# traveller59/spconv

Measured on NVIDIA H100. Metric: active-voxels/sec fwd+bwd SubMConv3d 3^3 C=64, higher is better.
Workload: dtype fp16

## Files before the change

spconv_b200/csrc/api_gemm.cu:

```cuda
#include "gemm.cuh"
#include "peer.cuh"
#include <stdlib.h>

using namespace spx;

namespace spx {
int write_tile_masks(const uint32_t *mask, int64_t rows, int kv, uint32_t *out, cudaStream_t stream);
}

static bool force_simt() { return runtime_cfg().force_simt != 0; }
static bool force_tc() { return runtime_cfg().force_tc != 0; }

static int check_desc(const spx_gemm_desc *d, const char *who) {
    SPX_REQUIRE(d != nullptr, "%s: descriptor is NULL", who);
    SPX_REQUIRE(d->kv >= 1 && d->kv <= 128, "%s: kernel volume %d not in [1,128]", who, d->kv);
    SPX_REQUIRE(d->c_in >= 1 && d->c_out >= 1, "%s: bad channel counts %d -> %d", who, d->c_in, d->c_out);
    SPX_REQUIRE(d->n_in >= 0 && d->n_out >= 0, "%s: negative row counts", who);
    SPX_REQUIRE(d->n_in < 2147483647ll && d->n_out < 2147483647ll, "%s: row counts must fit in int32", who);
    SPX_REQUIRE(d->pair != nullptr || (d->n_in == 0 || d->n_out == 0), "%s: pair table is NULL", who);
    SPX_REQUIRE((d->tile_table == nullptr) == (d->tile_mask == nullptr), "%s: tile_table and tile_mask go together", who);
    return 0;
}

static GatherGemmArgs make_args(const spx_gemm_desc *d, bool dgrad) {
    GatherGemmArgs a;
    memset(&a, 0, sizeof(a));
    a.dtype = d->dtype; a.f32_mode = d->f32_mode; a.kv = d->kv; a.c_in = d->c_in; a.c_out = d->c_out;
    a.transpose_w = dgrad ? 1 : 0;
    a.reverse = d->reverse_offsets;
    a.rows = dgrad ? d->n_in : d->n_out;
    a.x_rows = dgrad ? d->n_out : d->n_in;
    a.pair = d->pair; a.pair_stride = d->pair_stride;
    a.mask = d->mask; a.argsort = d->argsort;
    a.tile_table = d->tile_table; a.tile_mask = d->tile_mask;
    return a;
}

static int run_gather_gemm(const GatherGemmArgs &a, cudaStream_t stream) {
    if (a.rows == 0) return 0;
    bool exact_f32 = a.dtype == SPX_F32 && a.f32_mode == SPX_F32_EXACT;
    bool tc_ok = !force_simt() && !exact_f32 && tc_gather_gemm_supported(a);
    if (force_tc() && !tc_ok) {
        set_error("SPX_FORCE_TC=1 but the tensor-core path does not support this call (dtype %d, C %d, K %d)",
                  a.dtype, a.c_in, a.c_out);
        return 3;
    }
    if (tc_ok) { set_family(2); return tc_gather_gemm(a, stream); }
    set_family(1);
    return simt_gather_gemm(a, stream);
}

extern "C" int spx_implicit_gemm_fwd(const spx_gemm_desc *d, const void *features, const void *filters, void *out,
                                     const void *bias, int act, float act_alpha, uint32_t *mask_out,
                                     spx_stream_t stream) {
    if (check_desc(d, "implicit_gemm_fwd")) return 2;
    SPX_REQUIRE(d->dtype == SPX_F32 || d->dtype == SPX_F16 || d->dtype == SPX_BF16,
                "implicit_gemm_fwd: dtype %d not supported (int8 has its own entry point)", d->dtype);
    if (d->n_out == 0) return 0;
    SPX_REQUIRE(features && filters && out, "implicit_gemm_fwd: NULL tensor");
    GatherGemmArgs a = make_args(d, false);
    a.x = features; a.w = filters; a.y = out; a.bias = bias; a.act = act; a.alpha = act_alpha;
    a.mask_out = mask_out;
    return run_gather_gemm(a, (cudaStream_t)stream);
}

extern "C" int spx_implicit_gemm_dgrad(const spx_gemm_desc *d, const void *out_bp, const void *filters, void *din,
                                       spx_stream_t stream) {
    if (check_desc(d, "implicit_gemm_dgrad")) return 2;
    SPX_REQUIRE(d->dtype == SPX_F32 || d->dtype == SPX_F16 || d->dtype == SPX_BF16,
                "implicit_gemm_dgrad: dtype %d not supported", d->dtype);
    if (d->n_in == 0) return 0;
    SPX_REQUIRE(out_bp && filters && din, "implicit_gemm_dgrad: NULL tensor");
    GatherGemmArgs a = make_args(d, true);
    a.x = out_bp; a.w = filters; a.y = din; a.bias = nullptr; a.act = SPX_ACT_NONE;
    return run_gather_gemm(a, (cudaStream_t)stream);
}

static WgradArgs make_wgrad(const spx_gemm_desc *d) {
    WgradArgs w;
    memset(&w, 0, sizeof(w));
    w.dtype = d->dtype; w.f32_mode = d->f32_mode; w.kv = d->kv; w.c_in = d->c_in; w.c_out = d->c_out;
    w.n_in = d->n_in; w.n_out = d->n_out;
    w.pair = d->pair; w.pair_stride = d->pair_stride; w.mask = d->mask; w.argsort = d->argsort;
    w.tile_table = d->tile_table; w.tile_mask = d->tile_mask;
    return w;
}

extern "C" size_t spx_implicit_gemm_wgrad_workspace_size(const spx_gemm_desc *d) {
    if (!d) return 0;
    WgradArgs w = make_wgrad(d);
    bool exact_f32 = d->dtype == SPX_F32 && d->f32_mode == SPX_F32_EXACT;
    if (!force_simt() && !exact_f32 && tc_wgrad_supported(w)) return tc_wgrad_workspace_size(w);
    return 256;
}

static int wgrad_entry(const spx_gemm_desc *d, const void *features, const void *out_bp, void *dfilters, void *workspace,
                       size_t workspace_bytes, const spx_peer_group *pg, bool finish, float scale, spx_stream_t stream);

extern "C" int spx_implicit_gemm_wgrad(const spx_gemm_desc *d, const void *features, const void *out_bp,
                                       void *dfilters, void *workspace, size_t workspace_bytes,
                                       spx_stream_t stream) {
    return wgrad_entry(d, features, out_bp, dfilters, workspace, workspace_bytes, nullptr, false, 1.f, stream);
}

extern "C" int spx_implicit_gemm_wgrad_push(const spx_gemm_desc *d, const void *features, const void *out_bp,
                                            void *dfilters, void *workspace, size_t workspace_bytes,
                                            const spx_peer_group *pg, spx_stream_t stream) {
    SPX_REQUIRE(pg != nullptr, "implicit_gemm_wgrad_push: peer group is NULL");
    return wgrad_entry(d, features, out_bp, dfilters, workspace, workspace_bytes, pg, false, 1.f, stream);
}

extern "C" int spx_implicit_gemm_wgrad_allreduce(const spx_gemm_desc *d, const void *features, const void *out_bp,
                                                 void *dfilters, void *workspace, size_t workspace_bytes,
                                                 const spx_peer_group *pg, float scale, spx_stream_t stream) {
    SPX_REQUIRE(pg != nullptr, "implicit_gemm_wgrad_allreduce: peer group is NULL");
    return wgrad_entry(d, features, out_bp, dfilters, workspace, workspace_bytes, pg, true, scale, stream);
}

static int wgrad_entry(const spx_gemm_desc *d, const void *features, const void *out_bp, void *dfilters, void *workspace,
                       size_t workspace_bytes, const spx_peer_group *pg, bool finish, float scale, spx_stream_t stream) {
    if (check_desc(d, "implicit_gemm_wgrad")) return 2;
    SPX_REQUIRE(d->dtype == SPX_F32 || d->dtype == SPX_F16 || d->dtype == SPX_BF16,
                "implicit_gemm_wgrad: dtype %d not supported", d->dtype);
    SPX_REQUIRE(dfilters != nullptr, "implicit_gemm_wgrad: dfilters is NULL");
    const int64_t dw_count = (int64_t)d->kv * d->c_in * d->c_out;
    if (d->n_out == 0 || d->n_in == 0) {
        SPX_CHECK_CUDA(cudaMemsetAsync(dfilters, 0, (size_t)dw_count * dtype_bytes(d->dtype), (cudaStream_t)stream));
        if (pg) {
            if (int rc = peer_push(nullptr, 0, 0, dfilters, dw_count, d->dtype, pg, (cudaStream_t)stream)) return rc;
            if (finish) {
                return peer_finish(dfilters, dw_count, d->dtype, pg, scale, (cudaStream_t)stream);
            }
        }
        return 0;
    }
    SPX_REQUIRE(features && out_bp, "implicit_gemm_wgrad: NULL tensor");
    WgradArgs w = make_wgrad(d);
    w.peers = pg;
    w.x = features; w.dout = out_bp; w.dw = dfilters; w.workspace = workspace; w.workspace_bytes = workspace_bytes;
    bool exact_f32 = d->dtype == SPX_F32 && d->f32_mode == SPX_F32_EXACT;
    bool tc_ok = !force_simt() && !exact_f32 && tc_wgrad_supported(w);
    if (force_tc() && !tc_ok) {
        set_error("SPX_FORCE_TC=1 but the tensor-core wgrad does not support this call (dtype %d, C %d, K %d)", d->dtype,
                  d->c_in, d->c_out);
        return 3;
    }
    if (tc_ok) {
        SPX_REQUIRE(workspace && workspace_bytes >= tc_wgrad_workspace_size(w),
                    "implicit_gemm_wgrad: workspace too small (%zu < %zu)", workspace_bytes, tc_wgrad_workspace_size(w));
        set_family(2);
        if (int rc = tc_wgrad(w, (cudaStream_t)stream)) return rc;
        if (pg && finish) {
            return peer_finish(dfilters, dw_count, d->dtype, pg, scale, (cudaStream_t)stream);
        }
        return 0;
    }
    set_family(1);
    if (int rc = simt_wgrad(w, (cudaStream_t)stream)) return rc;
    if (pg) {
        if (int rc = peer_push(nullptr, 0, 0, dfilters, dw_count, d->dtype, pg, (cudaStream_t)stream)) return rc;
        if (finish) {
            return peer_finish(dfilters, dw_count, d->dtype, pg, scale, (cudaStream_t)stream);
        }
    }
    return 0;
}

extern "C" int spx_implicit_gemm_fwd_int8(const spx_gemm_desc *d, const int8_t *features, const int8_t *filters,
                                          void *out, int out_dtype, const float *scale, const float *bias,
                                          const int8_t *output_add, float output_add_scale, int act,
                                          float act_alpha, spx_stream_t stream) {
    if (check_desc(d, "implicit_gemm_fwd_int8")) return 2;
    SPX_REQUIRE(d->dtype == SPX_I8, "implicit_gemm_fwd_int8: descriptor dtype must be SPX_I8");
    SPX_REQUIRE(out_dtype == SPX_I8 || out_dtype == SPX_F32 || out_dtype == SPX_F16,
                "implicit_gemm_fwd_int8: out dtype %d not supported", out_dtype);
    if (d->n_out == 0) return 0;
    SPX_REQUIRE(features && filters && out && scale, "implicit_gemm_fwd_int8: NULL tensor");
    Int8Args q;
    memset(&q, 0, sizeof(q));
    q.g = make_args(d, false);
    q.g.x = features; q.g.w = filters; q.g.y = out; q.g.act = act; q.g.alpha = act_alpha;
    q.out_dtype = out_dtype; q.scale = scale; q.bias_f32 = bias; q.output_add = output_add;
    q.output_add_scale = output_add_scale;
    bool tc_ok = !force_simt() && tc_gather_gemm_int8_supported(q);
    if (force_tc() && !tc_ok) {
        set_error("SPX_FORCE_TC=1 but the tensor-core int8 path does not support C %d, K %d", d->c_in, d->c_out);
        return 3;
    }
    if (tc_ok) { set_family(2); return tc_gather_gemm_int8(q, (cudaStream_t)stream); }
    set_family(1);
    return simt_gather_gemm_int8(q, (cudaStream_t)stream);
}
```

spconv_b200/csrc/gemm.cuh:

```cuda
#pragma once
#include "common.cuh"

namespace spx {

struct GatherGemmArgs {
    int dtype, f32_mode, kv, c_in, c_out, transpose_w, reverse, act;
    float alpha;
    int64_t rows, x_rows;
    const void *x, *w, *bias;
    void *y;
    const int32_t *pair;
    int64_t pair_stride;
    const uint32_t *mask;
    const int32_t *argsort;
    uint32_t *mask_out;
    const int32_t *tile_table;
    const uint32_t *tile_mask;
    __host__ __device__ int cx() const { return transpose_w ? c_out : c_in; }
    __host__ __device__ int cy() const { return transpose_w ? c_in : c_out; }
};

struct WgradArgs {
    int dtype, f32_mode, kv, c_in, c_out;
    int64_t n_in, n_out;
    const void *x, *dout;
    void *dw;
    const int32_t *pair;
    int64_t pair_stride;
    const uint32_t *mask;
    const int32_t *argsort;
    const int32_t *tile_table;
    const uint32_t *tile_mask;
    void *workspace;
    size_t workspace_bytes;
    const spx_peer_group *peers;
};

constexpr int TT_REC_INTS = 8;
constexpr int TT_STATE_INTS = 64;
__host__ __device__ inline int64_t tt_blocks_elems(int64_t tiles, int kv) { return tiles * (int64_t)(kv + 1) * 128; }
__host__ __device__ inline int64_t tt_total_elems(int64_t tiles, int kv) {
    return tt_blocks_elems(tiles, kv) + tiles * TT_REC_INTS + TT_STATE_INTS;
}

int simt_gather_gemm(const GatherGemmArgs &a, cudaStream_t stream);
int simt_wgrad(const WgradArgs &a, cudaStream_t stream);

bool tc_gather_gemm_supported(const GatherGemmArgs &a);
int tc_gather_gemm(const GatherGemmArgs &a, cudaStream_t stream);
bool tc_wgrad_supported(const WgradArgs &a);
size_t tc_wgrad_workspace_size(const WgradArgs &a);
int tc_wgrad(const WgradArgs &a, cudaStream_t stream);

struct Int8Args {
    GatherGemmArgs g;
    int out_dtype;
    const float *scale, *bias_f32;
    const int8_t *output_add;
    float output_add_scale;
};
int simt_gather_gemm_int8(const Int8Args &a, cudaStream_t stream);
bool tc_gather_gemm_int8_supported(const Int8Args &a);
int tc_gather_gemm_int8(const Int8Args &a, cudaStream_t stream);

}
```

spconv_b200/csrc/gemm_tc_wgrad.cu:

```cuda
#include "gemm.cuh"
#include "peer.cuh"
#include "wgmma.cuh"
#include <stdlib.h>

namespace spx {

constexpr int WG_TILE = 128;
constexpr int WG_CONS_WARPS = 8;
constexpr int WG_PROD_WARPS = 2;
constexpr int WG_PROD_THREADS = WG_PROD_WARPS * 32;
constexpr int WG_SCHED_WARP = WG_CONS_WARPS + WG_PROD_WARPS;
constexpr int WG_THREADS = 3 * 128;
constexpr int WG_ACC_COLS = 256;
constexpr int WG_MAX_STAGES = 6;
constexpr int WG_SMEM_BUDGET = 200 * 1024;
constexpr int WG_SMEM_MAX = 224 * 1024;
constexpr int WG_MAX_IDX = 4;

struct WgParams {
    const uint8_t *x; int xb, span_x, lg_span_x, apo, apg, atom_elems;
    const uint8_t *d; int db, span_d, lg_span_d, lg_cpr_d;
    int n, ab_bf16;
    int groups_total, groups_per_pass;
    int stages, a_stage_bytes, b_buf_bytes, idx_bytes, idx_bufs;
    int64_t rows;
    const int32_t *tile_table;
    const uint32_t *tile_mask;
    const int32_t *sched_rec;
    int kv, words, c_in;
    float *partial; int64_t partial_stride;
    long long *dbg_ts;
    int debug;
};

__device__ __forceinline__ int slot_offset(int slot, int kv) {
    if (slot >= kv) return kv;
    return (slot & 1) ? kv - 1 - (slot >> 1) : (slot >> 1);
}

__device__ __forceinline__ uint32_t active_groups(const uint32_t (&tm)[4], const uint32_t *gmask, int ng, int words) {
    uint32_t act = 0;
    if (words == 1) {
        for (int gl = 0; gl < ng; ++gl) act |= (tm[0] & gmask[gl * 4]) ? 1u << gl : 0u;
        return act;
    }
    for (int gl = 0; gl < ng; ++gl) {
        const uint32_t hit = (tm[0] & gmask[gl * 4]) | (tm[1] & gmask[gl * 4 + 1]) | (tm[2] & gmask[gl * 4 + 2]) |
                             (tm[3] & gmask[gl * 4 + 3]);
        if (hit) act |= 1u << gl;
    }
    return act;
}

__device__ __forceinline__ int64_t wg_rec_index(int64_t i, int chunk, int chunks) {
    return i * chunks + ((i & 1) ? (chunks - 1 - chunk) : chunk);
}
__device__ __forceinline__ void wg_load_rec(const int32_t *__restrict__ rec, int64_t r, int64_t &tile, uint32_t (&m)[4]) {
    const int4 a = __ldg(reinterpret_cast<const int4 *>(rec + r * TT_REC_INTS));
    const int b = __ldg(rec + r * TT_REC_INTS + 4);
    tile = a.x; m[0] = (uint32_t)a.y; m[1] = (uint32_t)a.z; m[2] = (uint32_t)a.w; m[3] = (uint32_t)b;
}

__device__ __forceinline__ long long wg_global_ns() {
    long long t;
    asm volatile("mov.u64 %0, %%globaltimer;" : "=l"(t));
    return t;
}
#define WG_SPAN(i) do { if (p.dbg_ts && threadIdx.x == 0) { const int c_ = blockIdx.y * gridDim.x + blockIdx.x; if (c_ < 512) p.dbg_ts[2 * 2048 + c_ * 4 + (i)] = wg_global_ns(); } } while (0)

__device__ __forceinline__ uint32_t pick_word(const uint32_t (&m)[4], int w) {
    return w == 0 ? m[0] : (w == 1 ? m[1] : (w == 2 ? m[2] : m[3]));
}

__device__ __forceinline__ uint32_t kmajor_tf32_off(uint32_t row, uint32_t voxel, uint32_t rows) {
    return (voxel >> 5) * rows * 128u + swizzle_offset(row * 128u + ((voxel & 31u) << 2), 128u);
}
__device__ __forceinline__ void st_shared_f32x4_t(uint32_t base, uint32_t row0, uint32_t voxel, uint32_t rows, float4 v) {
    const float f[4] = {v.x, v.y, v.z, v.w};
#pragma unroll
    for (int t = 0; t < 4; ++t)
        asm volatile("st.shared.f32 [%0], %1;" ::"r"(base + kmajor_tf32_off(row0 + t, voxel, rows)), "f"(f[t]) : "memory");
}

template <int CPA, int CPD, bool TF32 = false>
__global__ void __launch_bounds__(WG_THREADS, 1)
tc_wgrad_kernel(const WgParams p) {
    constexpr int E = TF32 ? 4 : 2;
    constexpr int N = CPD * 16 / E;
    constexpr int G = WG_ACC_COLS / N < 16 ? WG_ACC_COLS / N : 16;
    constexpr int KSTEPS = WG_TILE * E / 32;
    constexpr int LG_CPA = CPA == 2 ? 1 : (CPA == 4 ? 2 : 3);
    constexpr int RPI = 32 / CPA;
    constexpr int LG_CPD = CPD == 2 ? 1 : (CPD == 4 ? 2 : (CPD == 8 ? 3 : (CPD == 16 ? 4 : 5)));
    constexpr int RPI_D = 32 / CPD;
    constexpr int DB = CPD * 16;
    constexpr int SPAN_D = DB < 128 ? DB : 128;
    constexpr int LG_SPAN_D = SPAN_D == 128 ? 7 : (SPAN_D == 64 ? 6 : 5);
    constexpr int SPAN_X = CPA * 16;
    constexpr int LG_SPAN_X = LG_CPA + 4;
    constexpr int ROWS_PW = WG_TILE / WG_PROD_WARPS;
    constexpr int ITERS = ROWS_PW / RPI > 0 ? ROWS_PW / RPI : 1;
    constexpr int ITERS_D = ROWS_PW / RPI_D;
    extern __shared__ __align__(1024) uint8_t smem_raw[];
    WG_SPAN(0);
    const uint32_t raw_addr = smem_u32(smem_raw);
    const uint32_t pad = (1024u - (raw_addr & 1023u)) & 1023u;
    uint8_t *smem = smem_raw + pad;
    const uint32_t smem_base = raw_addr + pad;
    const uint32_t b_base = smem_base;
    const uint32_t a_base = smem_base + 2u * p.b_buf_bytes;
    const uint32_t idx_off = 2u * p.b_buf_bytes + (uint32_t)p.stages * p.a_stage_bytes;
    uint64_t *bars = reinterpret_cast<uint64_t *>(smem + idx_off + (uint32_t)p.idx_bufs * p.idx_bytes);
    uint64_t *full_a = bars;
    uint64_t *empty_a = bars + WG_MAX_STAGES;
    uint64_t *full_b = bars + 2 * WG_MAX_STAGES;
    uint64_t *empty_b = bars + 2 * WG_MAX_STAGES + 2;
    uint64_t *idx_full = bars + 2 * WG_MAX_STAGES + 4;
    uint64_t *idx_empty = bars + 2 * WG_MAX_STAGES + 4 + WG_MAX_IDX;
    uint32_t *gmask = reinterpret_cast<uint32_t *>(bars + 2 * WG_MAX_STAGES + 4 + 2 * WG_MAX_IDX);
    uint32_t *slot_info = gmask + 32 * 4;

    const int warp = threadIdx.x >> 5;
    const int lane = threadIdx.x & 31;
    const int64_t num_tiles = (p.rows + WG_TILE - 1) / WG_TILE;
    const int chunk = blockIdx.x, chunks = gridDim.x;
    const int g_first = blockIdx.y, g_step = gridDim.y;
    const int ng = g_first < p.groups_total ? (p.groups_total - g_first + g_step - 1) / g_step : 0;

    if (threadIdx.x < 32) {
        const int g = g_first + (int)threadIdx.x * g_step;
        uint32_t m[4] = {0, 0, 0, 0};
        if ((int)threadIdx.x < ng) {
            for (int a = g * p.apg; a < (g + 1) * p.apg; ++a) {
                const int k = slot_offset(a / p.apo, p.kv);
                if (k < p.kv) m[k >> 5] |= 1u << (k & 31);
            }
        }
#pragma unroll
        for (int w = 0; w < 4; ++w) gmask[threadIdx.x * 4 + w] = m[w];
    }
    if (threadIdx.x == 0) {
        for (int s = 0; s < p.stages; ++s) { mbar_init(&full_a[s], WG_PROD_THREADS); mbar_init(&empty_a[s], WG_CONS_WARPS); }
        for (int b = 0; b < 2; ++b) { mbar_init(&full_b[b], WG_PROD_THREADS); mbar_init(&empty_b[b], WG_CONS_WARPS); }
        for (int b = 0; b < p.idx_bufs; ++b) { mbar_init(&idx_full[b], 1); mbar_init(&idx_empty[b], WG_PROD_WARPS); }
        mbar_fence_init();
    }
    __syncthreads();
    WG_SPAN(1);

    if (warp >= WG_CONS_WARPS && warp < WG_SCHED_WARP) {
        const int pw = warp - WG_CONS_WARPS;
        int stage = 0; uint32_t phase = 0;
        int64_t nb = 0;
        const int r0 = lane >> LG_CPA;
        const uint32_t chb = (uint32_t)(lane & (CPA - 1)) << 4;
        const uint8_t *x_lane = p.x + chb;
        uint32_t dst_off[ITERS];
#pragma unroll
        for (int itc = 0; itc < ITERS; ++itc)
            dst_off[itc] = swizzle_offset(((uint32_t)(pw * ROWS_PW + r0 + itc * RPI) << LG_SPAN_X) + chb, SPAN_X);
        const int lg_apo = p.apo == 1 ? 0 : (p.apo == 2 ? 1 : 2);
        const int rd0 = lane >> LG_CPD;
        const uint32_t chd = (uint32_t)(lane & (CPD - 1)) << 4;
        const uint8_t *d_lane = p.d + chd;
        const int nring = p.idx_bufs;
        auto issue_b = [&](const int32_t *idx_s) {
            const int bb = (int)(nb & 1);
            mbar_wait(&empty_b[bb], (uint32_t)(((nb >> 1) & 1) ^ 1));
            const uint32_t dstb = b_base + (uint32_t)bb * p.b_buf_bytes;
            const int32_t *rows_s = idx_s + p.kv * 128 + pw * ROWS_PW + rd0;
            int32_t rsrc[ITERS_D];
#pragma unroll
            for (int itc = 0; itc < ITERS_D; ++itc) rsrc[itc] = rows_s[itc * RPI_D];
            if constexpr (TF32) {
#pragma unroll 1
                for (int i0 = 0; i0 < ITERS_D; i0 += 8) {
                    float4 v[8];
#pragma unroll
                    for (int i = 0; i < 8; ++i) {
                        const int32_t r = i0 + i < ITERS_D ? rsrc[i0 + i] : -1;
                        v[i] = r >= 0 ? __ldg(reinterpret_cast<const float4 *>(d_lane + (int64_t)r * DB)) : make_float4(0.f, 0.f, 0.f, 0.f);
                    }
#pragma unroll
                    for (int i = 0; i < 8; ++i)
                        if (i0 + i < ITERS_D)
                            st_shared_f32x4_t(dstb, chd >> 2, (uint32_t)(pw * ROWS_PW + rd0 + (i0 + i) * RPI_D), (uint32_t)N, v[i]);
                }
                fence_proxy_async_smem();
                mbar_arrive(&full_b[bb]);
            } else {
#pragma unroll
                for (int itc = 0; itc < ITERS_D; ++itc) {
                    const uint32_t row_in_tile = (uint32_t)(pw * ROWS_PW + rd0 + itc * RPI_D);
                    const uint32_t off = (chd >> LG_SPAN_D) * (uint32_t)(WG_TILE * SPAN_D) +
                                         swizzle_offset((row_in_tile << LG_SPAN_D) + (chd & (uint32_t)(SPAN_D - 1)), SPAN_D);
                    cp_async_16(dstb + off, d_lane + (int64_t)max(rsrc[itc], 0) * DB, rsrc[itc] >= 0 ? 16u : 0u);
                }
                cp_async_mbar_arrive_noinc(&full_b[bb]);
            }
            ++nb;
        };
        auto idx_block = [&](int b) {
            return reinterpret_cast<const int32_t *>(smem + idx_off + (size_t)b * p.idx_bytes);
        };
        auto read_slot = [&](int slot, uint32_t use, uint32_t (&m)[4]) -> uint32_t {
            mbar_wait(&idx_full[slot], use & 1u);
            const volatile uint32_t *r = slot_info + slot * 8;
            m[0] = r[1]; m[1] = r[2]; m[2] = r[3]; m[3] = r[4];
            return r[0];
        };
        int cur_slot = 0; uint32_t cur_use = 0;
        uint32_t tm[4] = {0, 0, 0, 0}, tm1[4] = {0, 0, 0, 0};
        uint32_t act = 0;
        if (wg_rec_index(0, chunk, chunks) < num_tiles) {
            act = read_slot(0, 0u, tm);
            if (act) issue_b(idx_block(0));
        }
        for (int64_t step = 0; wg_rec_index(step, chunk, chunks) < num_tiles; ++step) {
            const bool has_next = wg_rec_index(step + 1, chunk, chunks) < num_tiles;
            int nxt_slot = cur_slot + 1; uint32_t nxt_use = cur_use;
            if (nxt_slot == nring) { nxt_slot = 0; ++nxt_use; }
            uint32_t act_next = 0;
            bool next_ready = !has_next;
            auto prepare_next = [&]() {
                act_next = read_slot(nxt_slot, nxt_use, tm1);
                if (act_next) issue_b(idx_block(nxt_slot));
                next_ready = true;
            };
            const int32_t *idx_s = idx_block(cur_slot);
            for (uint32_t rem = act; rem; rem &= rem - 1) {
                const int g = g_first + (__ffs(rem) - 1) * g_step;
                mbar_wait(&empty_a[stage], phase ^ 1u);
                const uint32_t a_stage = a_base + (uint32_t)stage * p.a_stage_bytes;
                for (int s = 0; s < p.apg; ++s) {
                    const int a = g * p.apg + s;
                    const int k = slot_offset(a >> lg_apo, p.kv);
                    const int cb = a & (p.apo - 1);
                    const bool active = k < p.kv && ((pick_word(tm, k >> 5) >> (k & 31)) & 1u);
                    const int32_t *idx_k = idx_s + (active ? k : 0) * 128 + pw * ROWS_PW + r0;
                    const uint8_t *x_atom = x_lane + cb * SPAN_X;
                    int32_t ridx[ITERS];
#pragma unroll
                    for (int itc = 0; itc < ITERS; ++itc) ridx[itc] = active ? idx_k[itc * RPI] : -1;
                    if constexpr (TF32) {
#pragma unroll
                        for (int itc = 0; itc < ITERS; ++itc) {
                            float4 v = make_float4(0.f, 0.f, 0.f, 0.f);
                            if (ridx[itc] >= 0) v = __ldg(reinterpret_cast<const float4 *>(x_atom + (int64_t)ridx[itc] * p.xb));
                            st_shared_f32x4_t(a_stage, (uint32_t)(s * 32) + (chb >> 2),
                                              (uint32_t)(pw * ROWS_PW + r0 + itc * RPI), (uint32_t)WG_TILE, v);
                        }
                    } else {
                        const uint32_t atom_base = a_stage + (uint32_t)s * (uint32_t)(WG_TILE * SPAN_X);
#pragma unroll
                        for (int itc = 0; itc < ITERS; ++itc)
                            cp_async_16(atom_base + dst_off[itc], x_atom + (int64_t)max(ridx[itc], 0) * p.xb,
                                        ridx[itc] >= 0 ? 16u : 0u);
                    }
                }
                if constexpr (TF32) {
                    fence_proxy_async_smem();
                    mbar_arrive(&full_a[stage]);
                } else {
                    cp_async_mbar_arrive_noinc(&full_a[stage]);
                }
                if (++stage == p.stages) { stage = 0; phase ^= 1u; }
                if (!next_ready) prepare_next();
            }
            if (!next_ready) prepare_next();
            __syncwarp();
            if (lane == 0) mbar_arrive(&idx_empty[cur_slot]);
#pragma unroll
            for (int w = 0; w < 4; ++w) tm[w] = tm1[w];
            act = act_next;
            cur_slot = nxt_slot; cur_use = nxt_use;
        }
    } else if (warp == WG_SCHED_WARP) {
        const uint32_t blk_bytes = (uint32_t)(p.kv + 1) * 512u;
        const int nring = p.idx_bufs;
        int slot = 0; uint32_t use = 0;
        uint32_t mw[4] = {0, 0, 0, 0};
        int64_t mtile = 0;
        for (int64_t i = 0; wg_rec_index(i, chunk, chunks) < num_tiles; ++i) {
            if ((i & 31) == 0) {
                const int64_t r = wg_rec_index(i + lane, chunk, chunks);
                if (r < num_tiles) wg_load_rec(p.sched_rec, r, mtile, mw);
            }
            uint32_t tm[4];
#pragma unroll
            for (int w = 0; w < 4; ++w) tm[w] = __shfl_sync(0xffffffffu, mw[w], (int)(i & 31));
            const int64_t tile = __shfl_sync(0xffffffffu, mtile, (int)(i & 31));
            const uint32_t act = active_groups(tm, gmask, ng, p.words);
            mbar_wait(&idx_empty[slot], (use & 1u) ^ 1u);
            if (lane == 0) {
                uint32_t *r = slot_info + slot * 8;
                r[0] = act; r[1] = tm[0]; r[2] = tm[1]; r[3] = tm[2]; r[4] = tm[3];
                if (act) {
                    mbar_arrive_expect_tx(&idx_full[slot], blk_bytes);
                    bulk_copy_g2s(smem_base + idx_off + (uint32_t)slot * p.idx_bytes,
                                  p.tile_table + tile * (int64_t)(p.kv + 1) * 128, blk_bytes, &idx_full[slot]);
                } else {
                    mbar_arrive(&idx_full[slot]);
                }
            }
            __syncwarp();
            if (++slot == nring) { slot = 0; ++use; }
        }
    } else if (warp < WG_CONS_WARPS) {
        const int wg = warp >> 2;
        int stage = 0; uint32_t phase = 0;
        int64_t nb = 0;
        uint32_t tm[4] = {0, 0, 0, 0};
        int64_t tile_unused = 0;
        if (wg_rec_index(0, chunk, chunks) < num_tiles)
            wg_load_rec(p.sched_rec, wg_rec_index(0, chunk, chunks), tile_unused, tm);
        const uint64_t a_hi = TF32 ? gmma_desc_hi(16u, 1024u, 128u)
                                   : gmma_desc_hi((uint32_t)(WG_TILE * SPAN_X), 8u * SPAN_X, SPAN_X);
        const uint64_t b_hi = TF32 ? gmma_desc_hi(16u, 1024u, 128u)
                                   : gmma_desc_hi((uint32_t)(WG_TILE * SPAN_D), 8u * SPAN_D, SPAN_D);
        const uint32_t a_wg = TF32 ? (uint32_t)wg * 64u * 128u : (uint32_t)wg * 64u * WG_TILE * E;
        float acc[G][N / 2];
#pragma unroll
        for (int gl = 0; gl < G; ++gl)
#pragma unroll
            for (int i = 0; i < N / 2; ++i) acc[gl][i] = 0.f;
        for (int64_t step = 0; wg_rec_index(step, chunk, chunks) < num_tiles; ++step) {
            const int64_t next = wg_rec_index(step + 1, chunk, chunks);
            uint32_t tm_next[4] = {0, 0, 0, 0};
            if (next < num_tiles) wg_load_rec(p.sched_rec, next, tile_unused, tm_next);
            const uint32_t act = active_groups(tm, gmask, ng, p.words);
            if (act) {
                const int bb = (int)(nb & 1);
                mbar_wait(&full_b[bb], (uint32_t)((nb >> 1) & 1));
                const uint32_t b16 = (b_base + (uint32_t)bb * p.b_buf_bytes) >> 4;
#pragma unroll
                for (int gl = 0; gl < G; ++gl) {
                    if (!((act >> gl) & 1u)) continue;
                    mbar_wait(&full_a[stage], phase);
                    fence_proxy_async_smem();
                    const uint32_t a16 = (a_base + (uint32_t)stage * p.a_stage_bytes + a_wg) >> 4;
                    fence_regs(acc[gl]);
                    wgmma_fence();
#pragma unroll
                    for (int j = 0; j < KSTEPS; ++j) {
                        if constexpr (TF32) {
                            const uint32_t ao = (uint32_t)(j >> 2) * (WG_TILE * 128u / 16u) + (uint32_t)(j & 3) * 2u;
                            const uint32_t bo = (uint32_t)(j >> 2) * (N * 128u / 16u) + (uint32_t)(j & 3) * 2u;
                            Wgmma<N>::tf32(acc[gl], a_hi | (uint64_t)((a16 + ao) & 0x3FFFu),
                                           b_hi | (uint64_t)((b16 + bo) & 0x3FFFu), 1u);
                        } else {
                            const uint64_t a_desc = a_hi | (uint64_t)((a16 + (uint32_t)j * SPAN_X) & 0x3FFFu);
                            const uint64_t b_desc = b_hi | (uint64_t)((b16 + (uint32_t)j * SPAN_D) & 0x3FFFu);
                            if (p.ab_bf16) Wgmma<N>::template bf16<1, 1>(acc[gl], a_desc, b_desc, 1u);
                            else Wgmma<N>::template f16<1, 1>(acc[gl], a_desc, b_desc, 1u);
                        }
                    }
                    wgmma_commit();
                    wgmma_wait<0>();
                    fence_regs(acc[gl]);
                    __syncwarp();
                    if (lane == 0) mbar_arrive(&empty_a[stage]);
                    if (++stage == p.stages) { stage = 0; phase ^= 1u; }
                }
                __syncwarp();
                if (lane == 0) mbar_arrive(&empty_b[bb]);
                ++nb;
            }
#pragma unroll
            for (int w = 0; w < 4; ++w) tm[w] = tm_next[w];
        }
        WG_SPAN(2);
        if (!(p.debug & 16)) {
            float *part = p.partial + (int64_t)chunk * p.partial_stride;
#pragma unroll
            for (int gl = 0; gl < G; ++gl) {
                if (gl >= ng) break;
                const int g = g_first + gl * g_step;
#pragma unroll
                for (int h = 0; h < 2; ++h) {
                    const int L = wg * 64 + (warp & 3) * 16 + (lane >> 2) + 8 * h;
                    const int s = L / p.atom_elems;
                    const int ce = L - s * p.atom_elems;
                    const int a = g * p.apg + s;
                    const int ks = a / p.apo;
                    const int k = slot_offset(ks, p.kv);
                    const int c = (a - ks * p.apo) * p.atom_elems + ce;
                    if (k >= p.kv) continue;
                    float *dst = part + (int64_t)k * p.c_in + c;
#pragma unroll
                    for (int nb8 = 0; nb8 < N / 8; ++nb8)
#pragma unroll
                        for (int j = 0; j < 2; ++j)
                            dst[(int64_t)(nb8 * 8 + 2 * (lane & 3) + j) * p.kv * p.c_in] = acc[gl][nb8 * 4 + 2 * h + j];
                }
            }
        }
    }

    __syncthreads();
    WG_SPAN(3);
}

constexpr int RED_WARPS = 8;
template <typename T>
__global__ void __launch_bounds__(RED_WARPS * 32)
wgrad_reduce_kernel(const float *__restrict__ partial, int64_t stride, int chunks, int64_t total,
                    T *__restrict__ dw) {
    __shared__ float4 acc_s[RED_WARPS][32];
    const int warp = threadIdx.x >> 5, lane = threadIdx.x & 31;
    const int64_t i = ((int64_t)blockIdx.x * 32 + lane) * 4;
    float4 s = make_float4(0.f, 0.f, 0.f, 0.f);
    if (i < total) {
        const int per = (chunks + RED_WARPS - 1) / RED_WARPS;
        const int c0 = warp * per, c1 = min(chunks, c0 + per);
#pragma unroll 4
        for (int c = c0; c < c1; ++c) {
            const float4 v = __ldg(reinterpret_cast<const float4 *>(partial + (int64_t)c * stride + i));
            s.x += v.x; s.y += v.y; s.z += v.z; s.w += v.w;
        }
    }
    acc_s[warp][lane] = s;
    __syncthreads();
    if (warp == 0 && i < total) {
        float4 t = acc_s[0][lane];
#pragma unroll
        for (int w = 1; w < RED_WARPS; ++w) {
            const float4 v = acc_s[w][lane];
            t.x += v.x; t.y += v.y; t.z += v.z; t.w += v.w;
        }
        dw[i] = from_float<T>(t.x); dw[i + 1] = from_float<T>(t.y);
        dw[i + 2] = from_float<T>(t.z); dw[i + 3] = from_float<T>(t.w);
    }
}

static bool wg_span_ok(int bytes) { return bytes == 32 || bytes == 64 || (bytes >= 128 && bytes % 128 == 0); }

struct WgPlan { WgParams p; int passes, chunks; size_t smem; };

static bool make_plan(const WgradArgs &a, WgPlan &pl) {
    if (a.dtype != SPX_F16 && a.dtype != SPX_BF16 && a.dtype != SPX_F32) return false;
    if (!a.tile_table || !a.tile_mask) return false;
    const bool tf32 = a.dtype == SPX_F32;
    const int e = tf32 ? 4 : 2;
    if (a.c_in % 16 || a.c_out % 16 || a.c_in > 256 || a.c_out > 256) return false;
    if (tf32 && (a.c_in % 32 || a.c_out % 32 || a.c_out > 128 || (runtime_cfg().debug & 4096))) return false;
    if (!wg_span_ok(a.c_in * e) || !wg_span_ok(a.c_out * e)) return false;
    WgParams &p = pl.p;
    memset(&p, 0, sizeof(p));
    p.xb = a.c_in * e; p.span_x = p.xb < 128 ? p.xb : 128;
    p.lg_span_x = p.span_x == 128 ? 7 : (p.span_x == 64 ? 6 : 5);
    p.apo = p.xb / p.span_x;
    p.atom_elems = p.span_x / e;
    p.apg = 128 / p.atom_elems;
    p.db = a.c_out * e; p.span_d = p.db < 128 ? p.db : 128;
    p.lg_span_d = p.span_d == 128 ? 7 : (p.span_d == 64 ? 6 : 5);
    if (p.db & (p.db - 1)) return false;
    p.lg_cpr_d = 0;
    while ((1 << p.lg_cpr_d) < (p.db >> 4)) ++p.lg_cpr_d;
    p.n = a.c_out;
    p.ab_bf16 = a.dtype == SPX_BF16;
    const int atoms_total = a.kv * p.apo;
    p.groups_total = (atoms_total + p.apg - 1) / p.apg;
    p.groups_per_pass = WG_ACC_COLS / a.c_out;
    if (p.groups_per_pass > 16) p.groups_per_pass = 16;
    if ((runtime_cfg().debug & 1024) && p.groups_per_pass >= 2) p.groups_per_pass /= 2;
    pl.passes = (p.groups_total + p.groups_per_pass - 1) / p.groups_per_pass;
    p.a_stage_bytes = p.apg * WG_TILE * p.span_x;
    p.b_buf_bytes = WG_TILE * p.db;
    p.idx_bytes = (int)align_up((size_t)(a.kv + 1) * 512, 1024);
    int avail = (tf32 ? WG_SMEM_MAX - 2048 : WG_SMEM_BUDGET) - 2 * p.b_buf_bytes - 2 * p.idx_bytes;
    if (avail < 2 * p.a_stage_bytes) return false;
    p.stages = avail / p.a_stage_bytes;
    if (p.stages > WG_MAX_STAGES) p.stages = WG_MAX_STAGES;
    size_t fixed = 2 * (size_t)p.b_buf_bytes + (size_t)p.stages * p.a_stage_bytes + 1024 + 1024;
    p.idx_bufs = 2;
    while (p.idx_bufs < WG_MAX_IDX && fixed + (size_t)(p.idx_bufs + 1) * p.idx_bytes <= (size_t)WG_SMEM_MAX) ++p.idx_bufs;
    pl.smem = fixed + (size_t)p.idx_bufs * p.idx_bytes;
    int64_t tiles = div_up64(a.n_out, WG_TILE);
    int chunks = sm_count() / pl.passes;
    if (chunks < 1) chunks = 1;
    if (chunks > tiles) chunks = (int)tiles;
    if (chunks < 1) chunks = 1;
    pl.chunks = chunks;
    p.rows = a.n_out; p.tile_table = a.tile_table; p.tile_mask = a.tile_mask;
    p.sched_rec = a.tile_table + tt_blocks_elems(tiles, a.kv);
    p.kv = a.kv; p.words = (a.kv + 31) / 32; p.c_in = a.c_in;
    p.x = (const uint8_t *)a.x; p.d = (const uint8_t *)a.dout;
    p.partial_stride = (int64_t)a.kv * a.c_in * a.c_out;
    return true;
}

bool tc_wgrad_supported(const WgradArgs &a) {
    WgPlan pl;
    return make_plan(a, pl);
}

size_t tc_wgrad_workspace_size(const WgradArgs &a) {
    WgPlan pl;
    if (!make_plan(a, pl)) return 256;
    return (size_t)pl.chunks * pl.p.partial_stride * sizeof(float) + 256;
}

int tc_wgrad(const WgradArgs &a, cudaStream_t stream) {
    WgPlan pl;
    SPX_REQUIRE(make_plan(a, pl), "tc_wgrad: unsupported shape");
    pl.p.partial = (float *)a.workspace;
    pl.p.dbg_ts = runtime_cfg().trace;
    pl.p.debug = runtime_cfg().debug;
    SPX_REQUIRE((size_t)pl.chunks * pl.p.partial_stride * sizeof(float) <= a.workspace_bytes,
                "tc_wgrad: workspace too small");
    SPX_REQUIRE(((uintptr_t)a.workspace & 15u) == 0, "tc_wgrad: workspace must be 16-byte aligned");
    dim3 grid(pl.chunks, pl.passes);
    const int cpa = pl.p.span_x >> 4, cpd = pl.p.db >> 4;
    using KernelFn = void (*)(const WgParams);
    KernelFn fn = nullptr;
    if (a.dtype == SPX_F32) {
        if (cpa == 8 && cpd == 8) fn = tc_wgrad_kernel<8, 8, true>;
        if (cpa == 8 && cpd == 16) fn = tc_wgrad_kernel<8, 16, true>;
        if (cpa == 8 && cpd == 32) fn = tc_wgrad_kernel<8, 32, true>;
    } else {
#define WG_PICK(A, D) if (cpa == A && cpd == D) fn = tc_wgrad_kernel<A, D>;
#define WG_PICK_ROW(A) WG_PICK(A, 2) WG_PICK(A, 4) WG_PICK(A, 8) WG_PICK(A, 16) WG_PICK(A, 32)
        WG_PICK_ROW(2) WG_PICK_ROW(4) WG_PICK_ROW(8)
#undef WG_PICK_ROW
#undef WG_PICK
    }
    SPX_REQUIRE(fn != nullptr, "tc_wgrad: no kernel instance for this channel layout");
    if (!func_configured((const void *)fn, current_device()))
        SPX_CHECK_CUDA(cudaFuncSetAttribute((const void *)fn, cudaFuncAttributeMaxDynamicSharedMemorySize,
                                            WG_SMEM_MAX));
    fn<<<grid, WG_THREADS, pl.smem, stream>>>(pl.p);
    SPX_CHECK_LAUNCH("tc_wgrad_kernel");
    const int64_t total = pl.p.partial_stride;
    if (a.peers)
        return peer_push(pl.p.partial, total, pl.chunks, nullptr, total, a.dtype, a.peers, stream);
    unsigned nblk = (unsigned)div_up64(total, 128);
    if (a.dtype == SPX_F32)
        wgrad_reduce_kernel<float><<<nblk, RED_WARPS * 32, 0, stream>>>(pl.p.partial, total, pl.chunks, total, (float *)a.dw);
    else if (a.dtype == SPX_F16)
        wgrad_reduce_kernel<__half><<<nblk, RED_WARPS * 32, 0, stream>>>(pl.p.partial, total, pl.chunks, total, (__half *)a.dw);
    else
        wgrad_reduce_kernel<__nv_bfloat16><<<nblk, RED_WARPS * 32, 0, stream>>>(pl.p.partial, total, pl.chunks, total, (__nv_bfloat16 *)a.dw);
    SPX_CHECK_LAUNCH("wgrad_reduce_kernel");
    return 0;
}

}
```

spconv_b200/csrc/peer.cu:

```cuda
#include "common.cuh"
#include "gemm.cuh"
#include "peer.cuh"

namespace spx {

constexpr size_t PEER_FLAGS = 256, PEER_DATA = 4096;

struct PeerState { unsigned epoch, finished, done, error; };

__device__ __forceinline__ void st_release_sys(unsigned *addr, unsigned v) {
    asm volatile("st.release.sys.global.u32 [%0], %1;" ::"l"(addr), "r"(v) : "memory");
}
__device__ __forceinline__ unsigned ld_acquire_sys(const unsigned *addr) {
    unsigned v;
    asm volatile("ld.acquire.sys.global.u32 %0, [%1];" : "=r"(v) : "l"(addr) : "memory");
    return v;
}
__device__ __forceinline__ unsigned long long globaltimer_ns() {
    unsigned long long t;
    asm volatile("mov.u64 %0, %globaltimer;" : "=l"(t));
    return t;
}

struct PeerPtrs { char *buf[SPX_MAX_PEERS]; };

constexpr int PX_THREADS = 256, PX_WARPS = PX_THREADS / 32;

template <typename T>
__global__ void __launch_bounds__(PX_THREADS)
peer_push_kernel(const float *__restrict__ partial, int64_t stride, int chunks, const T *__restrict__ src, int64_t total,
                 PeerPtrs peers, int world, int rank, int64_t capacity, int publish) {
    __shared__ float4 acc_s[PX_WARPS][32];
    __shared__ unsigned s_epoch;
    PeerState *st = reinterpret_cast<PeerState *>(peers.buf[rank]);
    if (threadIdx.x == 0) s_epoch = st->epoch;
    const int warp = threadIdx.x >> 5, lane = threadIdx.x & 31;
    const int64_t i = ((int64_t)blockIdx.x * 32 + lane) * 4;
    float4 s = make_float4(0.f, 0.f, 0.f, 0.f);
    if (partial) {
        if (i < total) {
            const int per = (chunks + PX_WARPS - 1) / PX_WARPS;
            const int c0 = warp * per, c1 = min(chunks, c0 + per);
#pragma unroll 4
            for (int c = c0; c < c1; ++c) {
                const float4 v = __ldg(reinterpret_cast<const float4 *>(partial + (int64_t)c * stride + i));
                s.x += v.x; s.y += v.y; s.z += v.z; s.w += v.w;
            }
        }
        acc_s[warp][lane] = s;
    }
    __syncthreads();
    if (warp != 0) return;
    const unsigned epoch = s_epoch;
    float4 t = make_float4(0.f, 0.f, 0.f, 0.f);
    if (partial) {
        t = acc_s[0][lane];
#pragma unroll
        for (int w = 1; w < PX_WARPS; ++w) {
            const float4 v = acc_s[w][lane];
            t.x += v.x; t.y += v.y; t.z += v.z; t.w += v.w;
        }
    } else if (i < total) {
        t.x = to_float<T>(src[i]);
        if (i + 1 < total) t.y = to_float<T>(src[i + 1]);
        if (i + 2 < total) t.z = to_float<T>(src[i + 2]);
        if (i + 3 < total) t.w = to_float<T>(src[i + 3]);
    }
    if (i < total)
        *reinterpret_cast<float4 *>(reinterpret_cast<float *>(peers.buf[rank] + PEER_DATA) + (int64_t)(epoch & 1u) * capacity + i) = t;
    if (!(publish & 1)) return;
    __threadfence();
    __syncwarp();
    unsigned last = 0;
    if (lane == 0) last = atomicAdd(&st->done, 1u) == gridDim.x - 1 ? 1u : 0u;
    last = __shfl_sync(0xffffffffu, last, 0);
    if (!last) return;
    if (publish & 2) {
        __threadfence();
        if (lane == 0) st->done = 0;
        if (lane < world)
            asm volatile("st.relaxed.sys.global.u32 [%0], %1;" ::"l"(reinterpret_cast<unsigned *>(peers.buf[lane] + PEER_FLAGS) + rank), "r"(epoch + 1u) : "memory");
        return;
    }
    __threadfence_system();
    if (lane == 0) st->done = 0;
    if (lane < world) st_release_sys(reinterpret_cast<unsigned *>(peers.buf[lane] + PEER_FLAGS) + rank, epoch + 1u);
}

constexpr int FIN_CHUNK_BYTES = 8192;
constexpr int FIN_MAX_CTAS = 64;

template <typename T>
__global__ void __launch_bounds__(PX_THREADS)
peer_finish_kernel(T *__restrict__ dst, int64_t total, PeerPtrs peers, int world, int rank, int64_t capacity, float scale,
                   unsigned long long timeout_ns, int publish) {
    extern __shared__ __align__(128) uint8_t fin_smem[];
    __shared__ __align__(8) uint64_t bar;
    __shared__ unsigned s_epoch;
    __shared__ int s_bad;
    char *mine = peers.buf[rank];
    PeerState *st = reinterpret_cast<PeerState *>(mine);
    if (threadIdx.x == 0) { s_epoch = st->epoch; s_bad = 0; mbar_init(&bar, 1); mbar_fence_init(); }
    __syncthreads();
    const unsigned epoch = s_epoch, target = epoch + 1u;
    if (publish && blockIdx.x == 0 && threadIdx.x < world) {
        __threadfence_system();
        st_release_sys(reinterpret_cast<unsigned *>(peers.buf[threadIdx.x] + PEER_FLAGS) + rank, target);
    }
    if (threadIdx.x < world) {
        const unsigned *flag = reinterpret_cast<const unsigned *>(mine + PEER_FLAGS) + threadIdx.x;
        const unsigned long long t0 = globaltimer_ns();
        unsigned spins = 0;
        while ((int)(ld_acquire_sys(flag) - target) < 0) {
            __nanosleep(200);
            if ((++spins & 255u) == 0 && globaltimer_ns() - t0 > timeout_ns) { s_bad = 1; break; }
        }
    }
    __syncthreads();
    const bool bad = s_bad != 0;
    if (bad && threadIdx.x == 0) st->error = 1u;
    const int64_t slot_off = (int64_t)(epoch & 1u) * capacity;
    const int64_t padded = (total + 3) / 4 * 4;
    const int64_t chunk_floats = FIN_CHUNK_BYTES / 4;
    const int64_t nchunks = (padded + chunk_floats - 1) / chunk_floats;
    const float nan = __int_as_float(0x7fc00000);
    uint32_t phase = 0;
    for (int64_t c = blockIdx.x; c < nchunks; c += gridDim.x) {
        const int64_t f0 = c * chunk_floats;
        const int nfl = (int)((padded - f0) < chunk_floats ? (padded - f0) : chunk_floats);
        if (threadIdx.x == 0) {
            asm volatile("fence.proxy.async;" ::: "memory");
            mbar_arrive_expect_tx(&bar, (uint32_t)(world * nfl * 4));
            for (int r = 0; r < world; ++r)
                bulk_copy_g2s(smem_u32(fin_smem + (size_t)r * FIN_CHUNK_BYTES),
                              reinterpret_cast<const float *>(peers.buf[r] + PEER_DATA) + slot_off + f0, (uint32_t)(nfl * 4), &bar);
        }
        mbar_wait(&bar, phase);
        phase ^= 1u;
        for (int j = threadIdx.x * 4; j < nfl; j += PX_THREADS * 4) {
            float4 t = *reinterpret_cast<const float4 *>(fin_smem + (size_t)j * 4);
            for (int r = 1; r < world; ++r) {
                const float4 v = *reinterpret_cast<const float4 *>(fin_smem + (size_t)r * FIN_CHUNK_BYTES + (size_t)j * 4);
                t.x += v.x; t.y += v.y; t.z += v.z; t.w += v.w;
            }
            if (bad) t = make_float4(nan, nan, nan, nan);
            const int64_t i = f0 + j;
            dst[i] = from_float<T>(t.x * scale);
            if (i + 1 < total) dst[i + 1] = from_float<T>(t.y * scale);
            if (i + 2 < total) dst[i + 2] = from_float<T>(t.z * scale);
            if (i + 3 < total) dst[i + 3] = from_float<T>(t.w * scale);
        }
        __syncthreads();
    }
    if (threadIdx.x == 0) {
        __threadfence();
        if (atomicAdd(&st->finished, 1u) == gridDim.x - 1) {
            st->finished = 0;
            st->epoch = epoch + 1;
            __threadfence();
        }
    }
}

static int check_group(const spx_peer_group *pg, int64_t total, const char *who) {
    SPX_REQUIRE(pg != nullptr, "%s: peer group is NULL", who);
    SPX_REQUIRE(pg->world >= 1 && pg->world <= SPX_MAX_PEERS && pg->rank >= 0 && pg->rank < pg->world,
                "%s: bad peer group (world %d, rank %d)", who, pg->world, pg->rank);
    SPX_REQUIRE(total >= 0 && (uint64_t)(total + 3) / 4 * 16 <= pg->capacity_bytes,
                "%s: %lld fp32 values exceed the exchange capacity of %llu bytes", who, (long long)total,
                (unsigned long long)pg->capacity_bytes);
    for (int r = 0; r < pg->world; ++r) SPX_REQUIRE(pg->buffers[r] != nullptr, "%s: buffer of rank %d is NULL", who, r);
    return 0;
}

static PeerPtrs peer_ptrs(const spx_peer_group *pg) {
    PeerPtrs pp;
    memset(&pp, 0, sizeof(pp));
    for (int r = 0; r < pg->world; ++r) pp.buf[r] = (char *)pg->buffers[r];
    return pp;
}
static unsigned push_ctas(int64_t total) { return (unsigned)div_up64(total, 128); }

int peer_push(const float *partial, int64_t stride, int chunks, const void *src, int64_t total, int dtype,
              const spx_peer_group *pg, cudaStream_t stream) {
    if (int rc = check_group(pg, total, "peer push")) return rc;
    if (total == 0) return 0;
    SPX_REQUIRE(!partial || total % 4 == 0, "peer push: partial sums need a multiple of 4 values");
    const PeerPtrs pp = peer_ptrs(pg);
    const int64_t cap = (int64_t)(pg->capacity_bytes / 4);
    const unsigned grid = push_ctas(total);
    const int publish = ((runtime_cfg().debug & 8192) ? 1 : 0) | ((runtime_cfg().debug & 16384) ? 2 : 0);
#define PX_LAUNCH(T) peer_push_kernel<T><<<grid, PX_THREADS, 0, stream>>>(partial, stride, chunks, (const T *)src, total, pp, pg->world, pg->rank, cap, publish)
    if (dtype == SPX_F16) PX_LAUNCH(__half);
    else if (dtype == SPX_BF16) PX_LAUNCH(__nv_bfloat16);
    else if (dtype == SPX_F32) PX_LAUNCH(float);
    else { set_error("peer push: dtype %d not supported", dtype); return 2; }
#undef PX_LAUNCH
    SPX_CHECK_LAUNCH("peer_push_kernel");
    return 0;
}

int peer_finish(void *dst, int64_t total, int dtype, const spx_peer_group *pg, float scale, cudaStream_t stream) {
    if (int rc = check_group(pg, total, "peer finish")) return rc;
    if (total == 0) return 0;
    const PeerPtrs pp = peer_ptrs(pg);
    const int64_t cap = (int64_t)(pg->capacity_bytes / 4);
    const int64_t nchunks = div_up64((total + 3) / 4 * 16, FIN_CHUNK_BYTES);
    int64_t max_ctas = FIN_MAX_CTAS;
    if (pg->colocated > 1 && max_ctas > FIN_MAX_CTAS / pg->colocated) max_ctas = FIN_MAX_CTAS / pg->colocated > 0 ? FIN_MAX_CTAS / pg->colocated : 1;
    const unsigned grid = (unsigned)(nchunks < max_ctas ? nchunks : max_ctas);
    const size_t smem = (size_t)pg->world * FIN_CHUNK_BYTES;
    const unsigned long long timeout_ns = (unsigned long long)(pg->timeout_ms > 0 ? pg->timeout_ms : 20000) * 1000000ull;
    const int publish = (runtime_cfg().debug & 8192) ? 0 : 1;
#define PX_LAUNCH(T)                                                                                                  \
    do {                                                                                                              \
        auto fn = peer_finish_kernel<T>;                                                                              \
        if (smem > 48 * 1024 && !func_configured((const void *)fn, current_device()))                                 \
            SPX_CHECK_CUDA(cudaFuncSetAttribute((const void *)fn, cudaFuncAttributeMaxDynamicSharedMemorySize,       \
                                                SPX_MAX_PEERS * FIN_CHUNK_BYTES));                                    \
        fn<<<grid, PX_THREADS, smem, stream>>>((T *)dst, total, pp, pg->world, pg->rank, cap, scale, timeout_ns, publish);      \
    } while (0)
    if (dtype == SPX_F16) PX_LAUNCH(__half);
    else if (dtype == SPX_BF16) PX_LAUNCH(__nv_bfloat16);
    else if (dtype == SPX_F32) PX_LAUNCH(float);
    else { set_error("peer finish: dtype %d not supported", dtype); return 2; }
#undef PX_LAUNCH
    SPX_CHECK_LAUNCH("peer_finish_kernel");
    return 0;
}

}

using namespace spx;

extern "C" size_t spx_peer_buffer_bytes(size_t capacity_bytes, int world) {
    if (world < 1 || world > SPX_MAX_PEERS) return 0;
    return PEER_DATA + 2 * align_up(capacity_bytes, 16);
}

extern "C" int spx_peer_buffer_create(size_t capacity_bytes, int world, void **buffer, unsigned char handle[64]) {
    SPX_REQUIRE(buffer && handle, "peer_buffer_create: NULL output");
    SPX_REQUIRE(world >= 1 && world <= SPX_MAX_PEERS, "peer_buffer_create: world %d out of range (1..%d)", world, SPX_MAX_PEERS);
    SPX_REQUIRE(capacity_bytes % 16 == 0 && capacity_bytes > 0, "peer_buffer_create: capacity must be a positive multiple of 16");
    static_assert(sizeof(cudaIpcMemHandle_t) == 64, "handle size");
    void *p = nullptr;
    const size_t bytes = spx_peer_buffer_bytes(capacity_bytes, world);
    SPX_CHECK_CUDA(cudaMalloc(&p, bytes));
    SPX_CHECK_CUDA(cudaMemset(p, 0, bytes));
    cudaIpcMemHandle_t h;
    cudaError_t e = cudaIpcGetMemHandle(&h, p);
    if (e != cudaSuccess) {
        cudaGetLastError();
        cudaFree(p);
        set_error("cudaIpcGetMemHandle failed: %s", cudaGetErrorString(e));
        return 1;
    }
    memcpy(handle, &h, 64);
    *buffer = p;
    return 0;
}

extern "C" int spx_peer_buffer_open(const unsigned char handle[64], void **mapped) {
    SPX_REQUIRE(handle && mapped, "peer_buffer_open: NULL argument");
    cudaIpcMemHandle_t h;
    memcpy(&h, handle, 64);
    SPX_CHECK_CUDA(cudaIpcOpenMemHandle(mapped, h, cudaIpcMemLazyEnablePeerAccess));
    return 0;
}

extern "C" int spx_peer_buffer_close(void *mapped) {
    if (mapped) SPX_CHECK_CUDA(cudaIpcCloseMemHandle(mapped));
    return 0;
}

extern "C" int spx_peer_buffer_destroy(void *buffer) {
    if (buffer) SPX_CHECK_CUDA(cudaFree(buffer));
    return 0;
}

extern "C" int spx_peer_error(const spx_peer_group *pg, int *error) {
    SPX_REQUIRE(pg && error, "peer_error: NULL argument");
    PeerState st;
    SPX_CHECK_CUDA(cudaMemcpy(&st, pg->buffers[pg->rank], sizeof(st), cudaMemcpyDeviceToHost));
    *error = (int)st.error;
    return 0;
}

extern "C" int spx_peer_push(const spx_peer_group *pg, const void *data, int64_t count, int dtype, spx_stream_t stream) {
    SPX_REQUIRE(data != nullptr || count == 0, "peer_push: data is NULL");
    return peer_push(nullptr, 0, 0, data, count, dtype, pg, (cudaStream_t)stream);
}

extern "C" int spx_peer_finish(const spx_peer_group *pg, void *out, int64_t count, int dtype, float scale,
                               spx_stream_t stream) {
    SPX_REQUIRE(out != nullptr || count == 0, "peer_finish: out is NULL");
    return peer_finish(out, count, dtype, pg, scale, (cudaStream_t)stream);
}

extern "C" int spx_peer_allreduce(const spx_peer_group *pg, void *data, int64_t count, int dtype, float scale,
                                  spx_stream_t stream) {
    if (int rc = spx_peer_push(pg, data, count, dtype, stream)) return rc;
    return spx_peer_finish(pg, data, count, dtype, scale, stream);
}
```

spconv_b200/csrc/peer.cuh:

```cuda
#pragma once
#include "common.cuh"

namespace spx {

int peer_push(const float *partial, int64_t stride, int chunks, const void *src, int64_t total, int dtype,
              const spx_peer_group *pg, cudaStream_t stream);
int peer_finish(void *dst, int64_t total, int dtype, const spx_peer_group *pg, float scale, cudaStream_t stream);

}
```

Before: 448.0 million.

## Plan wgrad CTA split in-kernel by cost and store compact per-CTA slabs

Replaces the fixed 2D grid (chunks × passes) for the tensor-core wgrad with a 1D grid where each CTA runs an in-kernel planning phase. The planner counts kernel-offset usage from the tile schedule, sorts offsets by frequency, estimates per-pass cost, and assigns CTAs to passes and row slices in proportion to that cost. Partial sums are now written as compact per-CTA slabs holding only the resident groups, plus a header that the reduce and peer-push kernels use to map each output element back. This aims to fix load imbalance across passes and shrink workspace and reduction traffic. In exchange every CTA repeats the planning scans over the tile records, which adds latency and complexity.

New measurement: 454.2 million, median of 6. Within noise of the previous version (+1.4%).

```diff
diff --git a/spconv_b200/csrc/api_gemm.cu b/spconv_b200/csrc/api_gemm.cu
--- a/spconv_b200/csrc/api_gemm.cu
+++ b/spconv_b200/csrc/api_gemm.cu
@@ -127,7 +127,7 @@
     if (d->n_out == 0 || d->n_in == 0) {
         SPX_CHECK_CUDA(cudaMemsetAsync(dfilters, 0, (size_t)dw_count * dtype_bytes(d->dtype), (cudaStream_t)stream));
         if (pg) {
-            if (int rc = peer_push(nullptr, 0, 0, dfilters, dw_count, d->dtype, pg, (cudaStream_t)stream)) return rc;
+            if (int rc = peer_push(nullptr, dfilters, dw_count, d->dtype, pg, (cudaStream_t)stream)) return rc;
             if (finish) {
                 return peer_finish(dfilters, dw_count, d->dtype, pg, scale, (cudaStream_t)stream);
             }
@@ -158,7 +158,7 @@
     set_family(1);
     if (int rc = simt_wgrad(w, (cudaStream_t)stream)) return rc;
     if (pg) {
-        if (int rc = peer_push(nullptr, 0, 0, dfilters, dw_count, d->dtype, pg, (cudaStream_t)stream)) return rc;
+        if (int rc = peer_push(nullptr, dfilters, dw_count, d->dtype, pg, (cudaStream_t)stream)) return rc;
         if (finish) {
             return peer_finish(dfilters, dw_count, d->dtype, pg, scale, (cudaStream_t)stream);
         }
diff --git a/spconv_b200/csrc/gemm.cuh b/spconv_b200/csrc/gemm.cuh
--- a/spconv_b200/csrc/gemm.cuh
+++ b/spconv_b200/csrc/gemm.cuh
@@ -43,6 +43,36 @@
     return tt_blocks_elems(tiles, kv) + tiles * TT_REC_INTS + TT_STATE_INTS;
 }
 
+constexpr int WG_HDR_FLOATS = 512;
+constexpr int WG_HDR_PASS = 128;
+struct WgSlabs {
+    const float *ws;
+    int kv, c_in, apo, atom_elems, apg;
+    int gpp, g_res;
+    int64_t slab;
+};
+__device__ __forceinline__ float4 wg_partial_sum(const WgSlabs &s, int64_t i, int part, int parts) {
+    const int32_t *hdr = reinterpret_cast<const int32_t *>(s.ws);
+    const int c = (int)(i % s.c_in);
+    const int64_t kn = i / s.c_in;
+    const int k = (int)(kn % s.kv);
+    const int64_t n = kn / s.kv;
+    const int a = __ldg(hdr + k) * s.apo + c / s.atom_elems;
+    const int g = a / s.apg, pass = g / s.gpp;
+    const int64_t off = (n * s.g_res + (g - pass * s.gpp)) * 128 + (a - g * s.apg) * s.atom_elems + c % s.atom_elems;
+    const int b = __ldg(hdr + WG_HDR_PASS + pass), e = __ldg(hdr + WG_HDR_PASS + pass + 1);
+    const int per = (e - b + parts - 1) / parts;
+    const int c0 = b + part * per, c1 = min(e, c0 + per);
+    const float *src = s.ws + WG_HDR_FLOATS + off;
+    float4 acc = make_float4(0.f, 0.f, 0.f, 0.f);
+#pragma unroll 4
+    for (int cta = c0; cta < c1; ++cta) {
+        const float4 v = __ldg(reinterpret_cast<const float4 *>(src + (int64_t)cta * s.slab));
+        acc.x += v.x; acc.y += v.y; acc.z += v.z; acc.w += v.w;
+    }
+    return acc;
+}
+
 int simt_gather_gemm(const GatherGemmArgs &a, cudaStream_t stream);
 int simt_wgrad(const WgradArgs &a, cudaStream_t stream);
 
diff --git a/spconv_b200/csrc/gemm_tc_wgrad.cu b/spconv_b200/csrc/gemm_tc_wgrad.cu
--- a/spconv_b200/csrc/gemm_tc_wgrad.cu
+++ b/spconv_b200/csrc/gemm_tc_wgrad.cu
@@ -17,26 +17,28 @@
 constexpr int WG_SMEM_MAX = 224 * 1024;
 constexpr int WG_MAX_IDX = 4;
 
+constexpr int WG_MAX_GROUPS = 256;
+constexpr int WG_PLAN_SCRATCH = 32 * 1024;
+constexpr int WG_PLAN_RB = 4;
+
+__host__ __device__ constexpr int wg_resident_groups(int n) { return WG_ACC_COLS / n < 16 ? WG_ACC_COLS / n : 16; }
+
 struct WgParams {
     const uint8_t *x; int xb, span_x, lg_span_x, apo, apg, atom_elems;
     const uint8_t *d; int db, span_d, lg_span_d, lg_cpr_d;
     int n, ab_bf16;
-    int groups_total, groups_per_pass;
+    int groups_total, groups_per_pass, passes;
     int stages, a_stage_bytes, b_buf_bytes, idx_bytes, idx_bufs;
+    int cost_stage, cost_tile;
     int64_t rows;
     const int32_t *tile_table;
     const uint32_t *tile_mask;
     const int32_t *sched_rec;
     int kv, words, c_in;
-    float *partial; int64_t partial_stride;
+    float *ws; int64_t slab;
     long long *dbg_ts;
     int debug;
 };
-
-__device__ __forceinline__ int slot_offset(int slot, int kv) {
-    if (slot >= kv) return kv;
-    return (slot & 1) ? kv - 1 - (slot >> 1) : (slot >> 1);
-}
 
 __device__ __forceinline__ uint32_t active_groups(const uint32_t (&tm)[4], const uint32_t *gmask, int ng, int words) {
     uint32_t act = 0;
@@ -52,8 +54,10 @@
     return act;
 }
 
-__device__ __forceinline__ int64_t wg_rec_index(int64_t i, int chunk, int chunks) {
-    return i * chunks + ((i & 1) ? (chunks - 1 - chunk) : chunk);
+__device__ __forceinline__ void wg_load_mask(const int32_t *__restrict__ rec, int64_t r, int words, uint32_t (&m)[4]) {
+    const int4 a = __ldg(reinterpret_cast<const int4 *>(rec + r * TT_REC_INTS));
+    m[0] = (uint32_t)a.y; m[1] = (uint32_t)a.z; m[2] = (uint32_t)a.w;
+    m[3] = words > 3 ? (uint32_t)__ldg(rec + r * TT_REC_INTS + 4) : 0u;
 }
 __device__ __forceinline__ void wg_load_rec(const int32_t *__restrict__ rec, int64_t r, int64_t &tile, uint32_t (&m)[4]) {
     const int4 a = __ldg(reinterpret_cast<const int4 *>(rec + r * TT_REC_INTS));
@@ -61,16 +65,294 @@
     tile = a.x; m[0] = (uint32_t)a.y; m[1] = (uint32_t)a.z; m[2] = (uint32_t)a.w; m[3] = (uint32_t)b;
 }
 
+__device__ __forceinline__ uint32_t pick_word(const uint32_t (&m)[4], int w) {
+    return w == 0 ? m[0] : (w == 1 ? m[1] : (w == 2 ? m[2] : m[3]));
+}
+
+__device__ __forceinline__ uint32_t wg_tile_cost(const WgParams &p, uint32_t act) {
+    return act ? (uint32_t)(__popc(act) * p.cost_stage + p.cost_tile) : 0u;
+}
+
+template <typename F>
+__device__ __forceinline__ void wg_walk(const WgParams &p, int rb, int re, const uint32_t *gmask, int ng, F &&f) {
+    const int lane = threadIdx.x & 31;
+    for (int r0 = rb; r0 < re; r0 += 32) {
+        uint32_t m[4] = {0, 0, 0, 0}, act = 0;
+        int64_t tile = 0;
+        if (r0 + lane < re) {
+            wg_load_rec(p.sched_rec, r0 + lane, tile, m);
+            act = active_groups(m, gmask, ng, p.words);
+        }
+        for (uint32_t live = __ballot_sync(0xffffffffu, act != 0); live; live &= live - 1) {
+            const int src = __ffs(live) - 1;
+            uint32_t tm[4];
+#pragma unroll
+            for (int w = 0; w < 4; ++w) tm[w] = __shfl_sync(0xffffffffu, m[w], src);
+            f(__shfl_sync(0xffffffffu, act, src), tm, __shfl_sync(0xffffffffu, tile, src));
+        }
+    }
+}
+
+
+__device__ __forceinline__ uint32_t plan_groups(const uint32_t (&m)[4], const uint32_t *gm, int ng) {
+    uint32_t act = 0;
+#pragma unroll 1
+    for (int gl = 0; gl < ng; ++gl) {
+        const uint4 g = *reinterpret_cast<const uint4 *>(gm + gl * 4);
+        act |= ((m[0] & g.x) | (m[1] & g.y) | (m[2] & g.z) | (m[3] & g.w)) ? 1u << gl : 0u;
+    }
+    return act;
+}
+
+__device__ __forceinline__ uint32_t warp_bit_counts(uint32_t p0, uint32_t p1, uint32_t p2, uint32_t *tp) {
+    const int lane = threadIdx.x & 31;
+    __syncwarp();
+    tp[lane] = p0; tp[32 + lane] = p1; tp[64 + lane] = p2;
+    __syncwarp();
+    uint32_t n = 0;
+#pragma unroll 8
+    for (int l = 0; l < 32; ++l)
+        n += ((tp[l] >> lane) & 1u) + ((tp[32 + l] >> lane) & 1u) * 2u + ((tp[64 + l] >> lane) & 1u) * 4u;
+    return n;
+}
+__device__ __forceinline__ void plane_add(uint32_t x, uint32_t &p0, uint32_t &p1, uint32_t &p2) {
+    const uint32_t c0 = p0 & x, c1 = p1 & c0;
+    p0 ^= x; p1 ^= c0; p2 |= c1;
+}
+
+__device__ __forceinline__ void wg_plan(const WgParams &p, uint8_t *scratch, uint8_t *slot_off, uint32_t *gmask,
+                                        int *walk) {
+    constexpr int NW = WG_THREADS / 32, RB = WG_PLAN_RB;
+    const int tid = threadIdx.x, lane = tid & 31, warp = tid >> 5;
+    const int T = (int)((p.rows + WG_TILE - 1) / WG_TILE);
+    const int gpp = p.groups_per_pass, passes = p.passes;
+    int *cnt = reinterpret_cast<int *>(scratch);
+    uint32_t *gm_all = reinterpret_cast<uint32_t *>(cnt + 128);
+    unsigned long long *pcost = reinterpret_cast<unsigned long long *>(gm_all + WG_MAX_GROUPS * 4);
+    unsigned long long *prem = pcost + WG_MAX_GROUPS;
+    int *pcta = reinterpret_cast<int *>(prem + WG_MAX_GROUPS);
+    uint32_t *wtot = reinterpret_cast<uint32_t *>(pcta + WG_MAX_GROUPS + 8);
+    int *slice = reinterpret_cast<int *>(wtot + NW);
+    uint32_t *tpw = reinterpret_cast<uint32_t *>(slice + 2) + warp * 96;
+    uint32_t *pm_all = reinterpret_cast<uint32_t *>(scratch + 16384);
+    int *gcnt = reinterpret_cast<int *>(pm_all + WG_MAX_GROUPS * 4);
+    int *pcnt = gcnt + WG_MAX_GROUPS;
+    auto load_batch = [&](int r0, int step, uint32_t (&b)[RB][4]) {
+#pragma unroll
+        for (int j = 0; j < RB; ++j) {
+            b[j][0] = b[j][1] = b[j][2] = b[j][3] = 0u;
+            if (r0 + j * step < T) wg_load_mask(p.sched_rec, r0 + j * step, p.words, b[j]);
+        }
+    };
+
+    if (tid < 128) cnt[tid] = 0;
+#pragma unroll 1
+    for (int i = tid; i < 2 * WG_MAX_GROUPS; i += WG_THREADS) gcnt[i] = 0;
+    if (tid < 2) slice[tid] = 0;
+    __syncthreads();
+    const int first_batch = warp * 32 * RB;
+    uint32_t bk[RB][4];
+    load_batch(first_batch + lane, 32, bk);
+    auto batch = [&](int r0, uint32_t (&b)[RB][4]) {
+        if (r0 == first_batch) {
+#pragma unroll
+            for (int j = 0; j < RB; ++j) {
+                b[j][0] = bk[j][0]; b[j][1] = bk[j][1]; b[j][2] = bk[j][2]; b[j][3] = bk[j][3];
+            }
+        } else {
+            load_batch(r0 + lane, 32, b);
+        }
+    };
+#pragma unroll 1
+    for (int r0 = first_batch; r0 < T; r0 += NW * 32 * RB) {
+        uint32_t b[RB][4];
+        batch(r0, b);
+#pragma unroll 1
+        for (int w = 0; w < p.words; ++w) {
+            uint32_t p0 = 0, p1 = 0, p2 = 0;
+#pragma unroll
+            for (int j = 0; j < RB; ++j) plane_add(pick_word(b[j], w), p0, p1, p2);
+            const uint32_t n = warp_bit_counts(p0, p1, p2, tpw);
+            if (w * 32 + lane < p.kv && n) atomicAdd(&cnt[w * 32 + lane], (int)n);
+        }
+    }
+    __syncthreads();
+    int my_slot = 0;
+    if (tid < p.kv) {
+        const int ck = cnt[tid];
+#pragma unroll 1
+        for (int j = 0; j < p.kv; ++j) {
+            const int cj = cnt[j];
+            my_slot += (cj > ck || (cj == ck && j < tid)) ? 1 : 0;
+        }
+    }
+    if (tid < 256) slot_off[tid] = (uint8_t)p.kv;
+    __syncthreads();
+    if (tid < p.kv) { slot_off[my_slot] = (uint8_t)tid; cnt[tid] = my_slot; }
+    __syncthreads();
+    if (tid < p.groups_total) {
+        uint32_t m0 = 0, m1 = 0, m2 = 0, m3 = 0;
+#pragma unroll 1
+        for (int a = tid * p.apg; a < (tid + 1) * p.apg; ++a) {
+            const int k = slot_off[a / p.apo];
+            const uint32_t bit = k < p.kv ? 1u << (k & 31) : 0u;
+            m0 |= (k >> 5) == 0 ? bit : 0u; m1 |= (k >> 5) == 1 ? bit : 0u;
+            m2 |= (k >> 5) == 2 ? bit : 0u; m3 |= (k >> 5) == 3 ? bit : 0u;
+        }
+        *reinterpret_cast<uint4 *>(gm_all + tid * 4) = make_uint4(m0, m1, m2, m3);
+    }
+    __syncthreads();
+    if (tid < passes) {
+        uint4 u = make_uint4(0u, 0u, 0u, 0u);
+#pragma unroll 1
+        for (int g = tid * gpp; g < min((tid + 1) * gpp, p.groups_total); ++g) {
+            const uint4 v = *reinterpret_cast<const uint4 *>(gm_all + g * 4);
+            u.x |= v.x; u.y |= v.y; u.z |= v.z; u.w |= v.w;
+        }
+        *reinterpret_cast<uint4 *>(pm_all + tid * 4) = u;
+    }
+    __syncthreads();
+    {
+        const int gcols = (p.groups_total + 31) >> 5, cols = gcols + ((passes + 31) >> 5);
+#pragma unroll 1
+        for (int r0 = first_batch; r0 < T; r0 += NW * 32 * RB) {
+            uint32_t b[RB][4];
+            batch(r0, b);
+#pragma unroll 1
+            for (int col = 0; col < cols; ++col) {
+                const bool grp = col < gcols;
+                const int c0 = (grp ? col : col - gcols) * 32;
+                const int nc = min(32, (grp ? p.groups_total : passes) - c0);
+                const uint4 *msk = reinterpret_cast<const uint4 *>(grp ? gm_all : pm_all) + c0;
+                uint32_t x[RB] = {0u, 0u, 0u, 0u};
+#pragma unroll 2
+                for (int c = 0; c < nc; ++c) {
+                    const uint4 g = msk[c];
+#pragma unroll
+                    for (int j = 0; j < RB; ++j)
+                        x[j] |= ((b[j][0] & g.x) | (b[j][1] & g.y) | (b[j][2] & g.z) | (b[j][3] & g.w)) ? 1u << c : 0u;
+                }
+                uint32_t p0 = 0, p1 = 0, p2 = 0;
+#pragma unroll
+                for (int j = 0; j < RB; ++j) plane_add(x[j], p0, p1, p2);
+                const uint32_t n = warp_bit_counts(p0, p1, p2, tpw);
+                if (lane < nc && n) atomicAdd(grp ? &gcnt[c0 + lane] : &pcnt[c0 + lane], (int)n);
+            }
+        }
+    }
+    __syncthreads();
+    if (tid < passes) {
+        unsigned long long stages = 0;
+#pragma unroll 1
+        for (int g = tid * gpp; g < min((tid + 1) * gpp, p.groups_total); ++g) stages += (unsigned)gcnt[g];
+        pcost[tid] = stages * (unsigned)p.cost_stage + (unsigned long long)(unsigned)pcnt[tid] * (unsigned)p.cost_tile;
+    }
+    __syncthreads();
+    unsigned long long total = 0;
+    int working = 0;
+#pragma unroll 1
+    for (int ps = 0; ps < passes; ++ps) { total += pcost[ps]; working += pcost[ps] ? 1 : 0; }
+    const unsigned long long spare = (unsigned long long)((int)gridDim.x - working);
+    int n = 0;
+    unsigned long long rem = 0;
+    if (tid < passes && pcost[tid]) {
+        const unsigned long long q = spare * pcost[tid];
+        n = 1 + (int)(q / total);
+        rem = q % total;
+    }
+    if (tid < passes) { pcta[tid] = n; prem[tid] = rem; }
+    __syncthreads();
+    int left = (int)gridDim.x;
+#pragma unroll 1
+    for (int ps = 0; ps < passes; ++ps) left -= pcta[ps];
+    if (tid < passes && pcost[tid]) {
+        int rank = 0;
+#pragma unroll 1
+        for (int ps = 0; ps < passes; ++ps)
+            rank += (pcost[ps] && (prem[ps] > rem || (prem[ps] == rem && ps < tid))) ? 1 : 0;
+        if (rank < left) ++n;
+    }
+    __syncthreads();
+    if (tid < passes) pcta[tid] = n;
+    __syncthreads();
+    if (tid == 0) {
+        int first = 0;
+#pragma unroll 1
+        for (int ps = 0; ps < passes; ++ps) { const int k = pcta[ps]; pcta[ps] = first; first += k; }
+        pcta[passes] = first;
+    }
+    __syncthreads();
+    if (blockIdx.x == 0) {
+        int32_t *hdr = reinterpret_cast<int32_t *>(p.ws);
+        if (tid < p.kv) hdr[tid] = cnt[tid];
+        if (tid <= passes) hdr[WG_HDR_PASS + tid] = pcta[tid];
+    }
+    int pass = -1;
+#pragma unroll 1
+    for (int ps = 0; ps < passes; ++ps)
+        if ((int)blockIdx.x >= pcta[ps] && (int)blockIdx.x < pcta[ps + 1]) pass = ps;
+    if (pass < 0) {
+        if (tid == 0) walk[0] = -1;
+        __syncthreads();
+        return;
+    }
+    const int ng = min(gpp, p.groups_total - pass * gpp);
+    if (tid < 16 * 4) gmask[tid] = tid < ng * 4 ? gm_all[pass * gpp * 4 + tid] : 0u;
+    __syncthreads();
+    const int j = (int)blockIdx.x - pcta[pass], ctas = pcta[pass + 1] - pcta[pass];
+    const unsigned long long lo = (unsigned long long)j * pcost[pass], hi = lo + pcost[pass];
+    unsigned long long carry = 0;
+#pragma unroll 1
+    for (int base = 0; base < T; base += NW * 32 * RB) {
+        const int r0 = base + first_batch;
+        uint32_t b[RB][4];
+        batch(r0, b);
+        uint32_t c[RB], ex[RB], wsum = 0;
+#pragma unroll
+        for (int i = 0; i < RB; ++i) {
+            c[i] = wg_tile_cost(p, plan_groups(b[i], gmask, ng));
+            uint32_t inc = c[i];
+#pragma unroll
+            for (int o = 1; o < 32; o <<= 1) {
+                const uint32_t up = __shfl_up_sync(0xffffffffu, inc, o);
+                if (lane >= o) inc += up;
+            }
+            ex[i] = wsum + inc - c[i];
+            wsum += __shfl_sync(0xffffffffu, inc, 31);
+        }
+        if (lane == 0) wtot[warp] = wsum;
+        __syncthreads();
+        unsigned long long s0 = carry, all = 0;
+#pragma unroll 1
+        for (int w = 0; w < NW; ++w) {
+            if (w < warp) s0 += wtot[w];
+            all += wtot[w];
+        }
+        uint32_t before = 0, upto = 0;
+#pragma unroll
+        for (int i = 0; i < RB; ++i) {
+            const unsigned long long sn = (s0 + ex[i]) * (unsigned long long)ctas;
+            const bool ok = r0 + i * 32 + lane < T;
+            before += (ok && sn < lo) ? 1u : 0u;
+            upto += (ok && sn < hi) ? 1u : 0u;
+        }
+        before = __reduce_add_sync(0xffffffffu, before);
+        upto = __reduce_add_sync(0xffffffffu, upto);
+        if (lane == 0) { atomicAdd(&slice[0], (int)before); atomicAdd(&slice[1], (int)upto); }
+        carry += all;
+        __syncthreads();
+    }
+    if (tid == 0) { walk[0] = pass; walk[1] = slice[0]; walk[2] = slice[1]; }
+    __syncthreads();
+}
+
 __device__ __forceinline__ long long wg_global_ns() {
     long long t;
     asm volatile("mov.u64 %0, %%globaltimer;" : "=l"(t));
     return t;
 }
-#define WG_SPAN(i) do { if (p.dbg_ts && threadIdx.x == 0) { const int c_ = blockIdx.y * gridDim.x + blockIdx.x; if (c_ < 512) p.dbg_ts[2 * 2048 + c_ * 4 + (i)] = wg_global_ns(); } } while (0)
-
-__device__ __forceinline__ uint32_t pick_word(const uint32_t (&m)[4], int w) {
-    return w == 0 ? m[0] : (w == 1 ? m[1] : (w == 2 ? m[2] : m[3]));
-}
+#define WG_SPAN(i) do { if (p.dbg_ts && threadIdx.x == 0 && blockIdx.x < 512) p.dbg_ts[2 * 2048 + blockIdx.x * 4 + (i)] = wg_global_ns(); } while (0)
+
 
 __device__ __forceinline__ uint32_t kmajor_tf32_off(uint32_t row, uint32_t voxel, uint32_t rows) {
     return (voxel >> 5) * rows * 128u + swizzle_offset(row * 128u + ((voxel & 31u) << 2), 128u);
@@ -87,7 +369,7 @@
 tc_wgrad_kernel(const WgParams p) {
     constexpr int E = TF32 ? 4 : 2;
     constexpr int N = CPD * 16 / E;
-    constexpr int G = WG_ACC_COLS / N < 16 ? WG_ACC_COLS / N : 16;
+    constexpr int G = wg_resident_groups(N);
     constexpr int KSTEPS = WG_TILE * E / 32;
     constexpr int LG_CPA = CPA == 2 ? 1 : (CPA == 4 ? 2 : 3);
     constexpr int RPI = 32 / CPA;
@@ -118,27 +400,18 @@
     uint64_t *idx_full = bars + 2 * WG_MAX_STAGES + 4;
     uint64_t *idx_empty = bars + 2 * WG_MAX_STAGES + 4 + WG_MAX_IDX;
     uint32_t *gmask = reinterpret_cast<uint32_t *>(bars + 2 * WG_MAX_STAGES + 4 + 2 * WG_MAX_IDX);
-    uint32_t *slot_info = gmask + 32 * 4;
+    uint32_t *slot_info = gmask + 16 * 4;
+    uint8_t *slot_off = reinterpret_cast<uint8_t *>(slot_info + WG_MAX_IDX * 8);
+    int *walk = reinterpret_cast<int *>(slot_off + 256);
 
     const int warp = threadIdx.x >> 5;
     const int lane = threadIdx.x & 31;
-    const int64_t num_tiles = (p.rows + WG_TILE - 1) / WG_TILE;
-    const int chunk = blockIdx.x, chunks = gridDim.x;
-    const int g_first = blockIdx.y, g_step = gridDim.y;
-    const int ng = g_first < p.groups_total ? (p.groups_total - g_first + g_step - 1) / g_step : 0;
-
-    if (threadIdx.x < 32) {
-        const int g = g_first + (int)threadIdx.x * g_step;
-        uint32_t m[4] = {0, 0, 0, 0};
-        if ((int)threadIdx.x < ng) {
-            for (int a = g * p.apg; a < (g + 1) * p.apg; ++a) {
-                const int k = slot_offset(a / p.apo, p.kv);
-                if (k < p.kv) m[k >> 5] |= 1u << (k & 31);
-            }
-        }
-#pragma unroll
-        for (int w = 0; w < 4; ++w) gmask[threadIdx.x * 4 + w] = m[w];
-    }
+    wg_plan(p, smem + 2u * p.b_buf_bytes, slot_off, gmask, walk);
+    const volatile int *walk_v = walk;
+    if (walk_v[0] < 0) return;
+    const int g_first = walk_v[0] * p.groups_per_pass;
+    const int ng = min(p.groups_per_pass, p.groups_total - g_first);
+
     if (threadIdx.x == 0) {
         for (int s = 0; s < p.stages; ++s) { mbar_init(&full_a[s], WG_PROD_THREADS); mbar_init(&empty_a[s], WG_CONS_WARPS); }
         for (int b = 0; b < 2; ++b) { mbar_init(&full_b[b], WG_PROD_THREADS); mbar_init(&empty_b[b], WG_CONS_WARPS); }
@@ -211,17 +484,13 @@
         };
         int cur_slot = 0; uint32_t cur_use = 0;
         uint32_t tm[4] = {0, 0, 0, 0}, tm1[4] = {0, 0, 0, 0};
-        uint32_t act = 0;
-        if (wg_rec_index(0, chunk, chunks) < num_tiles) {
-            act = read_slot(0, 0u, tm);
-            if (act) issue_b(idx_block(0));
-        }
-        for (int64_t step = 0; wg_rec_index(step, chunk, chunks) < num_tiles; ++step) {
-            const bool has_next = wg_rec_index(step + 1, chunk, chunks) < num_tiles;
+        uint32_t act = read_slot(0, 0u, tm);
+        if (act) issue_b(idx_block(0));
+        while (act) {
             int nxt_slot = cur_slot + 1; uint32_t nxt_use = cur_use;
             if (nxt_slot == nring) { nxt_slot = 0; ++nxt_use; }
             uint32_t act_next = 0;
-            bool next_ready = !has_next;
+            bool next_ready = false;
             auto prepare_next = [&]() {
                 act_next = read_slot(nxt_slot, nxt_use, tm1);
                 if (act_next) issue_b(idx_block(nxt_slot));
@@ -229,12 +498,12 @@
             };
             const int32_t *idx_s = idx_block(cur_slot);
             for (uint32_t rem = act; rem; rem &= rem - 1) {
-                const int g = g_first + (__ffs(rem) - 1) * g_step;
+                const int g = g_first + __ffs(rem) - 1;
                 mbar_wait(&empty_a[stage], phase ^ 1u);
                 const uint32_t a_stage = a_base + (uint32_t)stage * p.a_stage_bytes;
                 for (int s = 0; s < p.apg; ++s) {
                     const int a = g * p.apg + s;
-                    const int k = slot_offset(a >> lg_apo, p.kv);
+                    const int k = slot_off[a >> lg_apo];
                     const int cb = a & (p.apo - 1);
                     const bool active = k < p.kv && ((pick_word(tm, k >> 5) >> (k & 31)) & 1u);
                     const int32_t *idx_k = idx_s + (active ? k : 0) * 128 + pw * ROWS_PW + r0;
@@ -279,18 +548,7 @@
         const uint32_t blk_bytes = (uint32_t)(p.kv + 1) * 512u;
         const int nring = p.idx_bufs;
         int slot = 0; uint32_t use = 0;
-        uint32_t mw[4] = {0, 0, 0, 0};
-        int64_t mtile = 0;
-        for (int64_t i = 0; wg_rec_index(i, chunk, chunks) < num_tiles; ++i) {
-            if ((i & 31) == 0) {
-                const int64_t r = wg_rec_index(i + lane, chunk, chunks);
-                if (r < num_tiles) wg_load_rec(p.sched_rec, r, mtile, mw);
-            }
-            uint32_t tm[4];
-#pragma unroll
-            for (int w = 0; w < 4; ++w) tm[w] = __shfl_sync(0xffffffffu, mw[w], (int)(i & 31));
-            const int64_t tile = __shfl_sync(0xffffffffu, mtile, (int)(i & 31));
-            const uint32_t act = active_groups(tm, gmask, ng, p.words);
+        auto publish = [&](uint32_t act, const uint32_t (&tm)[4], int64_t tile) {
             mbar_wait(&idx_empty[slot], (use & 1u) ^ 1u);
             if (lane == 0) {
                 uint32_t *r = slot_info + slot * 8;
@@ -305,15 +563,14 @@
             }
             __syncwarp();
             if (++slot == nring) { slot = 0; ++use; }
-        }
+        };
+        wg_walk(p, walk_v[1], walk_v[2], gmask, ng, publish);
+        const uint32_t none[4] = {0, 0, 0, 0};
+        publish(0u, none, 0);
     } else if (warp < WG_CONS_WARPS) {
         const int wg = warp >> 2;
         int stage = 0; uint32_t phase = 0;
         int64_t nb = 0;
-        uint32_t tm[4] = {0, 0, 0, 0};
-        int64_t tile_unused = 0;
-        if (wg_rec_index(0, chunk, chunks) < num_tiles)
-            wg_load_rec(p.sched_rec, wg_rec_index(0, chunk, chunks), tile_unused, tm);
         const uint64_t a_hi = TF32 ? gmma_desc_hi(16u, 1024u, 128u)
                                    : gmma_desc_hi((uint32_t)(WG_TILE * SPAN_X), 8u * SPAN_X, SPAN_X);
         const uint64_t b_hi = TF32 ? gmma_desc_hi(16u, 1024u, 128u)
@@ -324,74 +581,57 @@
         for (int gl = 0; gl < G; ++gl)
 #pragma unroll
             for (int i = 0; i < N / 2; ++i) acc[gl][i] = 0.f;
-        for (int64_t step = 0; wg_rec_index(step, chunk, chunks) < num_tiles; ++step) {
-            const int64_t next = wg_rec_index(step + 1, chunk, chunks);
-            uint32_t tm_next[4] = {0, 0, 0, 0};
-            if (next < num_tiles) wg_load_rec(p.sched_rec, next, tile_unused, tm_next);
-            const uint32_t act = active_groups(tm, gmask, ng, p.words);
-            if (act) {
-                const int bb = (int)(nb & 1);
-                mbar_wait(&full_b[bb], (uint32_t)((nb >> 1) & 1));
-                const uint32_t b16 = (b_base + (uint32_t)bb * p.b_buf_bytes) >> 4;
-#pragma unroll
-                for (int gl = 0; gl < G; ++gl) {
-                    if (!((act >> gl) & 1u)) continue;
-                    mbar_wait(&full_a[stage], phase);
-                    fence_proxy_async_smem();
-                    const uint32_t a16 = (a_base + (uint32_t)stage * p.a_stage_bytes + a_wg) >> 4;
-                    fence_regs(acc[gl]);
-                    wgmma_fence();
-#pragma unroll
-                    for (int j = 0; j < KSTEPS; ++j) {
-                        if constexpr (TF32) {
-                            const uint32_t ao = (uint32_t)(j >> 2) * (WG_TILE * 128u / 16u) + (uint32_t)(j & 3) * 2u;
-                            const uint32_t bo = (uint32_t)(j >> 2) * (N * 128u / 16u) + (uint32_t)(j & 3) * 2u;
-                            Wgmma<N>::tf32(acc[gl], a_hi | (uint64_t)((a16 + ao) & 0x3FFFu),
-                                           b_hi | (uint64_t)((b16 + bo) & 0x3FFFu), 1u);
-                        } else {
-                            const uint64_t a_desc = a_hi | (uint64_t)((a16 + (uint32_t)j * SPAN_X) & 0x3FFFu);
-                            const uint64_t b_desc = b_hi | (uint64_t)((b16 + (uint32_t)j * SPAN_D) & 0x3FFFu);
-                            if (p.ab_bf16) Wgmma<N>::template bf16<1, 1>(acc[gl], a_desc, b_desc, 1u);
-                            else Wgmma<N>::template f16<1, 1>(acc[gl], a_desc, b_desc, 1u);
-                        }
+        wg_walk(p, walk_v[1], walk_v[2], gmask, ng, [&](uint32_t act, const uint32_t (&)[4], int64_t) {
+            const int bb = (int)(nb & 1);
+            mbar_wait(&full_b[bb], (uint32_t)((nb >> 1) & 1));
+            const uint32_t b16 = (b_base + (uint32_t)bb * p.b_buf_bytes) >> 4;
+#pragma unroll
+            for (int gl = 0; gl < G; ++gl) {
+                if (!((act >> gl) & 1u)) continue;
+                mbar_wait(&full_a[stage], phase);
+                fence_proxy_async_smem();
+                const uint32_t a16 = (a_base + (uint32_t)stage * p.a_stage_bytes + a_wg) >> 4;
+                fence_regs(acc[gl]);
+                wgmma_fence();
+#pragma unroll
+                for (int j = 0; j < KSTEPS; ++j) {
+                    if constexpr (TF32) {
+                        const uint32_t ao = (uint32_t)(j >> 2) * (WG_TILE * 128u / 16u) + (uint32_t)(j & 3) * 2u;
+                        const uint32_t bo = (uint32_t)(j >> 2) * (N * 128u / 16u) + (uint32_t)(j & 3) * 2u;
+                        Wgmma<N>::tf32(acc[gl], a_hi | (uint64_t)((a16 + ao) & 0x3FFFu),
+                                       b_hi | (uint64_t)((b16 + bo) & 0x3FFFu), 1u);
+                    } else {
+                        const uint64_t a_desc = a_hi | (uint64_t)((a16 + (uint32_t)j * SPAN_X) & 0x3FFFu);
+                        const uint64_t b_desc = b_hi | (uint64_t)((b16 + (uint32_t)j * SPAN_D) & 0x3FFFu);
+                        if (p.ab_bf16) Wgmma<N>::template bf16<1, 1>(acc[gl], a_desc, b_desc, 1u);
+                        else Wgmma<N>::template f16<1, 1>(acc[gl], a_desc, b_desc, 1u);
                     }
-                    wgmma_commit();
-                    wgmma_wait<0>();
-                    fence_regs(acc[gl]);
-                    __syncwarp();
-                    if (lane == 0) mbar_arrive(&empty_a[stage]);
-                    if (++stage == p.stages) { stage = 0; phase ^= 1u; }
                 }
+                wgmma_commit();
+                wgmma_wait<0>();
+                fence_regs(acc[gl]);
                 __syncwarp();
-                if (lane == 0) mbar_arrive(&empty_b[bb]);
-                ++nb;
+                if (lane == 0) mbar_arrive(&empty_a[stage]);
+                if (++stage == p.stages) { stage = 0; phase ^= 1u; }
             }
-#pragma unroll
-            for (int w = 0; w < 4; ++w) tm[w] = tm_next[w];
-        }
+            __syncwarp();
+            if (lane == 0) mbar_arrive(&empty_b[bb]);
+            ++nb;
+        });
         WG_SPAN(2);
         if (!(p.debug & 16)) {
-            float *part = p.partial + (int64_t)chunk * p.partial_stride;
+            float *part = p.ws + WG_HDR_FLOATS + (int64_t)blockIdx.x * p.slab + 2 * (lane & 3) * (G * WG_TILE);
 #pragma unroll
             for (int gl = 0; gl < G; ++gl) {
                 if (gl >= ng) break;
-                const int g = g_first + gl * g_step;
 #pragma unroll
                 for (int h = 0; h < 2; ++h) {
-                    const int L = wg * 64 + (warp & 3) * 16 + (lane >> 2) + 8 * h;
-                    const int s = L / p.atom_elems;
-                    const int ce = L - s * p.atom_elems;
-                    const int a = g * p.apg + s;
-                    const int ks = a / p.apo;
-                    const int k = slot_offset(ks, p.kv);
-                    const int c = (a - ks * p.apo) * p.atom_elems + ce;
-                    if (k >= p.kv) continue;
-                    float *dst = part + (int64_t)k * p.c_in + c;
+                    float *dst = part + gl * WG_TILE + wg * 64 + (warp & 3) * 16 + (lane >> 2) + 8 * h;
 #pragma unroll
                     for (int nb8 = 0; nb8 < N / 8; ++nb8)
 #pragma unroll
                         for (int j = 0; j < 2; ++j)
-                            dst[(int64_t)(nb8 * 8 + 2 * (lane & 3) + j) * p.kv * p.c_in] = acc[gl][nb8 * 4 + 2 * h + j];
+                            dst[(nb8 * 8 + j) * (G * WG_TILE)] = acc[gl][nb8 * 4 + 2 * h + j];
                 }
             }
         }
@@ -404,21 +644,11 @@
 constexpr int RED_WARPS = 8;
 template <typename T>
 __global__ void __launch_bounds__(RED_WARPS * 32)
-wgrad_reduce_kernel(const float *__restrict__ partial, int64_t stride, int chunks, int64_t total,
-                    T *__restrict__ dw) {
+wgrad_reduce_kernel(const WgSlabs slabs, int64_t total, T *__restrict__ dw) {
     __shared__ float4 acc_s[RED_WARPS][32];
     const int warp = threadIdx.x >> 5, lane = threadIdx.x & 31;
     const int64_t i = ((int64_t)blockIdx.x * 32 + lane) * 4;
-    float4 s = make_float4(0.f, 0.f, 0.f, 0.f);
-    if (i < total) {
-        const int per = (chunks + RED_WARPS - 1) / RED_WARPS;
-        const int c0 = warp * per, c1 = min(chunks, c0 + per);
-#pragma unroll 4
-        for (int c = c0; c < c1; ++c) {
-            const float4 v = __ldg(reinterpret_cast<const float4 *>(partial + (int64_t)c * stride + i));
-            s.x += v.x; s.y += v.y; s.z += v.z; s.w += v.w;
-        }
-    }
+    const float4 s = i < total ? wg_partial_sum(slabs, i, warp, RED_WARPS) : make_float4(0.f, 0.f, 0.f, 0.f);
     acc_s[warp][lane] = s;
     __syncthreads();
     if (warp == 0 && i < total) {
@@ -435,14 +665,14 @@
 
 static bool wg_span_ok(int bytes) { return bytes == 32 || bytes == 64 || (bytes >= 128 && bytes % 128 == 0); }
 
-struct WgPlan { WgParams p; int passes, chunks; size_t smem; };
+struct WgPlan { WgParams p; int ctas; size_t smem; };
 
 static bool make_plan(const WgradArgs &a, WgPlan &pl) {
     if (a.dtype != SPX_F16 && a.dtype != SPX_BF16 && a.dtype != SPX_F32) return false;
     if (!a.tile_table || !a.tile_mask) return false;
     const bool tf32 = a.dtype == SPX_F32;
     const int e = tf32 ? 4 : 2;
-    if (a.c_in % 16 || a.c_out % 16 || a.c_in > 256 || a.c_out > 256) return false;
+    if (a.c_in % 16 || a.c_out % 16 || a.c_in > 256 || a.c_out > 256 || a.kv < 1 || a.kv > 128) return false;
     if (tf32 && (a.c_in % 32 || a.c_out % 32 || a.c_out > 128 || (runtime_cfg().debug & 4096))) return false;
     if (!wg_span_ok(a.c_in * e) || !wg_span_ok(a.c_out * e)) return false;
     WgParams &p = pl.p;
@@ -461,10 +691,10 @@
     p.ab_bf16 = a.dtype == SPX_BF16;
     const int atoms_total = a.kv * p.apo;
     p.groups_total = (atoms_total + p.apg - 1) / p.apg;
-    p.groups_per_pass = WG_ACC_COLS / a.c_out;
-    if (p.groups_per_pass > 16) p.groups_per_pass = 16;
+    p.groups_per_pass = wg_resident_groups(a.c_out);
     if ((runtime_cfg().debug & 1024) && p.groups_per_pass >= 2) p.groups_per_pass /= 2;
-    pl.passes = (p.groups_total + p.groups_per_pass - 1) / p.groups_per_pass;
+    p.passes = (p.groups_total + p.groups_per_pass - 1) / p.groups_per_pass;
+    if (p.groups_total > WG_MAX_GROUPS) return false;
     p.a_stage_bytes = p.apg * WG_TILE * p.span_x;
     p.b_buf_bytes = WG_TILE * p.db;
     p.idx_bytes = (int)align_up((size_t)(a.kv + 1) * 512, 1024);
@@ -472,21 +702,20 @@
     if (avail < 2 * p.a_stage_bytes) return false;
     p.stages = avail / p.a_stage_bytes;
     if (p.stages > WG_MAX_STAGES) p.stages = WG_MAX_STAGES;
+    if (p.stages * p.a_stage_bytes < WG_PLAN_SCRATCH) return false;
+    p.cost_stage = p.a_stage_bytes / 512;
+    p.cost_tile = (p.b_buf_bytes + (a.kv + 1) * 512) / 512;
     size_t fixed = 2 * (size_t)p.b_buf_bytes + (size_t)p.stages * p.a_stage_bytes + 1024 + 1024;
     p.idx_bufs = 2;
     while (p.idx_bufs < WG_MAX_IDX && fixed + (size_t)(p.idx_bufs + 1) * p.idx_bytes <= (size_t)WG_SMEM_MAX) ++p.idx_bufs;
     pl.smem = fixed + (size_t)p.idx_bufs * p.idx_bytes;
     int64_t tiles = div_up64(a.n_out, WG_TILE);
-    int chunks = sm_count() / pl.passes;
-    if (chunks < 1) chunks = 1;
-    if (chunks > tiles) chunks = (int)tiles;
-    if (chunks < 1) chunks = 1;
-    pl.chunks = chunks;
+    pl.ctas = sm_count() > p.passes ? sm_count() : p.passes;
     p.rows = a.n_out; p.tile_table = a.tile_table; p.tile_mask = a.tile_mask;
     p.sched_rec = a.tile_table + tt_blocks_elems(tiles, a.kv);
     p.kv = a.kv; p.words = (a.kv + 31) / 32; p.c_in = a.c_in;
     p.x = (const uint8_t *)a.x; p.d = (const uint8_t *)a.dout;
-    p.partial_stride = (int64_t)a.kv * a.c_in * a.c_out;
+    p.slab = (int64_t)wg_resident_groups(a.c_out) * WG_TILE * a.c_out;
     return true;
 }
 
@@ -498,19 +727,19 @@
 size_t tc_wgrad_workspace_size(const WgradArgs &a) {
     WgPlan pl;
     if (!make_plan(a, pl)) return 256;
-    return (size_t)pl.chunks * pl.p.partial_stride * sizeof(float) + 256;
+    return (WG_HDR_FLOATS + (size_t)pl.ctas * pl.p.slab) * sizeof(float);
 }
 
 int tc_wgrad(const WgradArgs &a, cudaStream_t stream) {
     WgPlan pl;
     SPX_REQUIRE(make_plan(a, pl), "tc_wgrad: unsupported shape");
-    pl.p.partial = (float *)a.workspace;
+    pl.p.ws = (float *)a.workspace;
     pl.p.dbg_ts = runtime_cfg().trace;
     pl.p.debug = runtime_cfg().debug;
-    SPX_REQUIRE((size_t)pl.chunks * pl.p.partial_stride * sizeof(float) <= a.workspace_bytes,
+    SPX_REQUIRE((WG_HDR_FLOATS + (size_t)pl.ctas * pl.p.slab) * sizeof(float) <= a.workspace_bytes,
                 "tc_wgrad: workspace too small");
     SPX_REQUIRE(((uintptr_t)a.workspace & 15u) == 0, "tc_wgrad: workspace must be 16-byte aligned");
-    dim3 grid(pl.chunks, pl.passes);
+    const unsigned grid = (unsigned)pl.ctas;
     const int cpa = pl.p.span_x >> 4, cpd = pl.p.db >> 4;
     using KernelFn = void (*)(const WgParams);
     KernelFn fn = nullptr;
@@ -531,16 +760,18 @@
                                             WG_SMEM_MAX));
     fn<<<grid, WG_THREADS, pl.smem, stream>>>(pl.p);
     SPX_CHECK_LAUNCH("tc_wgrad_kernel");
-    const int64_t total = pl.p.partial_stride;
+    const int64_t total = (int64_t)a.kv * a.c_in * a.c_out;
+    const WgSlabs slabs{pl.p.ws, a.kv, a.c_in, pl.p.apo, pl.p.atom_elems, pl.p.apg, pl.p.groups_per_pass,
+                        wg_resident_groups(a.c_out), pl.p.slab};
     if (a.peers)
-        return peer_push(pl.p.partial, total, pl.chunks, nullptr, total, a.dtype, a.peers, stream);
+        return peer_push(&slabs, nullptr, total, a.dtype, a.peers, stream);
     unsigned nblk = (unsigned)div_up64(total, 128);
     if (a.dtype == SPX_F32)
-        wgrad_reduce_kernel<float><<<nblk, RED_WARPS * 32, 0, stream>>>(pl.p.partial, total, pl.chunks, total, (float *)a.dw);
+        wgrad_reduce_kernel<float><<<nblk, RED_WARPS * 32, 0, stream>>>(slabs, total, (float *)a.dw);
     else if (a.dtype == SPX_F16)
-        wgrad_reduce_kernel<__half><<<nblk, RED_WARPS * 32, 0, stream>>>(pl.p.partial, total, pl.chunks, total, (__half *)a.dw);
+        wgrad_reduce_kernel<__half><<<nblk, RED_WARPS * 32, 0, stream>>>(slabs, total, (__half *)a.dw);
     else
-        wgrad_reduce_kernel<__nv_bfloat16><<<nblk, RED_WARPS * 32, 0, stream>>>(pl.p.partial, total, pl.chunks, total, (__nv_bfloat16 *)a.dw);
+        wgrad_reduce_kernel<__nv_bfloat16><<<nblk, RED_WARPS * 32, 0, stream>>>(slabs, total, (__nv_bfloat16 *)a.dw);
     SPX_CHECK_LAUNCH("wgrad_reduce_kernel");
     return 0;
 }
diff --git a/spconv_b200/csrc/peer.cu b/spconv_b200/csrc/peer.cu
--- a/spconv_b200/csrc/peer.cu
+++ b/spconv_b200/csrc/peer.cu
@@ -28,7 +28,7 @@
 
 template <typename T>
 __global__ void __launch_bounds__(PX_THREADS)
-peer_push_kernel(const float *__restrict__ partial, int64_t stride, int chunks, const T *__restrict__ src, int64_t total,
+peer_push_kernel(const WgSlabs slabs, const T *__restrict__ src, int64_t total,
                  PeerPtrs peers, int world, int rank, int64_t capacity, int publish) {
     __shared__ float4 acc_s[PX_WARPS][32];
     __shared__ unsigned s_epoch;
@@ -36,19 +36,9 @@
     if (threadIdx.x == 0) s_epoch = st->epoch;
     const int warp = threadIdx.x >> 5, lane = threadIdx.x & 31;
     const int64_t i = ((int64_t)blockIdx.x * 32 + lane) * 4;
-    float4 s = make_float4(0.f, 0.f, 0.f, 0.f);
-    if (partial) {
-        if (i < total) {
-            const int per = (chunks + PX_WARPS - 1) / PX_WARPS;
-            const int c0 = warp * per, c1 = min(chunks, c0 + per);
-#pragma unroll 4
-            for (int c = c0; c < c1; ++c) {
-                const float4 v = __ldg(reinterpret_cast<const float4 *>(partial + (int64_t)c * stride + i));
-                s.x += v.x; s.y += v.y; s.z += v.z; s.w += v.w;
-            }
-        }
-        acc_s[warp][lane] = s;
-    }
+    const bool partial = slabs.ws != nullptr;
+    if (partial)
+        acc_s[warp][lane] = i < total ? wg_partial_sum(slabs, i, warp, PX_WARPS) : make_float4(0.f, 0.f, 0.f, 0.f);
     __syncthreads();
     if (warp != 0) return;
     const unsigned epoch = s_epoch;
@@ -181,16 +171,19 @@
 }
 static unsigned push_ctas(int64_t total) { return (unsigned)div_up64(total, 128); }
 
-int peer_push(const float *partial, int64_t stride, int chunks, const void *src, int64_t total, int dtype,
-              const spx_peer_group *pg, cudaStream_t stream) {
+int peer_push(const WgSlabs *slabs, const void *src, int64_t total, int dtype, const spx_peer_group *pg,
+              cudaStream_t stream) {
     if (int rc = check_group(pg, total, "peer push")) return rc;
     if (total == 0) return 0;
-    SPX_REQUIRE(!partial || total % 4 == 0, "peer push: partial sums need a multiple of 4 values");
+    SPX_REQUIRE(!slabs || total % 4 == 0, "peer push: partial sums need a multiple of 4 values");
     const PeerPtrs pp = peer_ptrs(pg);
     const int64_t cap = (int64_t)(pg->capacity_bytes / 4);
     const unsigned grid = push_ctas(total);
     const int publish = ((runtime_cfg().debug & 8192) ? 1 : 0) | ((runtime_cfg().debug & 16384) ? 2 : 0);
-#define PX_LAUNCH(T) peer_push_kernel<T><<<grid, PX_THREADS, 0, stream>>>(partial, stride, chunks, (const T *)src, total, pp, pg->world, pg->rank, cap, publish)
+    WgSlabs none;
+    memset(&none, 0, sizeof(none));
+    const WgSlabs sl = slabs ? *slabs : none;
+#define PX_LAUNCH(T) peer_push_kernel<T><<<grid, PX_THREADS, 0, stream>>>(sl, (const T *)src, total, pp, pg->world, pg->rank, cap, publish)
     if (dtype == SPX_F16) PX_LAUNCH(__half);
     else if (dtype == SPX_BF16) PX_LAUNCH(__nv_bfloat16);
     else if (dtype == SPX_F32) PX_LAUNCH(float);
@@ -288,7 +281,7 @@
 
 extern "C" int spx_peer_push(const spx_peer_group *pg, const void *data, int64_t count, int dtype, spx_stream_t stream) {
     SPX_REQUIRE(data != nullptr || count == 0, "peer_push: data is NULL");
-    return peer_push(nullptr, 0, 0, data, count, dtype, pg, (cudaStream_t)stream);
+    return peer_push(nullptr, data, count, dtype, pg, (cudaStream_t)stream);
 }
 
 extern "C" int spx_peer_finish(const spx_peer_group *pg, void *out, int64_t count, int dtype, float scale,
diff --git a/spconv_b200/csrc/peer.cuh b/spconv_b200/csrc/peer.cuh
--- a/spconv_b200/csrc/peer.cuh
+++ b/spconv_b200/csrc/peer.cuh
@@ -3,8 +3,9 @@
 
 namespace spx {
 
-int peer_push(const float *partial, int64_t stride, int chunks, const void *src, int64_t total, int dtype,
-              const spx_peer_group *pg, cudaStream_t stream);
+struct WgSlabs;
+int peer_push(const WgSlabs *slabs, const void *src, int64_t total, int dtype, const spx_peer_group *pg,
+              cudaStream_t stream);
 int peer_finish(void *dst, int64_t total, int dtype, const spx_peer_group *pg, float scale, cudaStream_t stream);
 
 }
```
